# lmdu/pyfastx

Measured on NVIDIA B200. Metric: index_build_GBps, higher is better.
Workload: dtype u8

## Files before the change

pyfastx_b200/csrc/fxg_api.cu:

```cuda
#include "fxg_common.cuh"
#include <stdarg.h>
#include <stdlib.h>
#include <string.h>
#include <fcntl.h>
#include <unistd.h>
#include <sys/stat.h>
#include <sched.h>
#include <sys/mman.h>
#include <sys/syscall.h>
#include <thread>
#include <vector>
#include <atomic>
#include <mutex>

static thread_local char g_err[512] = "";

void fxg_set_error(const char *fmt, ...) {
    va_list ap;
    va_start(ap, fmt);
    vsnprintf(g_err, sizeof(g_err), fmt, ap);
    va_end(ap);
}

void fxg_pool_drain(int device);

int FxgScratch::reserve(size_t bytes) {
    if (bytes <= cap) return FXG_OK;
    if (ptr) cudaFree(ptr);
    ptr = nullptr; cap = 0;
    size_t want = bytes + bytes / 8 + 4096;
    cudaError_t e = cudaMalloc(&ptr, want);
    if (e != cudaSuccess) {
        cudaGetLastError();
        int dev = 0;
        cudaGetDevice(&dev);
        fxg_pool_drain(dev);
        want = bytes;
        e = cudaMalloc(&ptr, want);
    }
    if (e != cudaSuccess) {
        cudaGetLastError();
        ptr = nullptr;
        fxg_set_error("cudaMalloc(%zu) failed: %s", bytes, cudaGetErrorString(e));
        return FXG_ENOMEM;
    }
    cap = want;
    return FXG_OK;
}
void FxgScratch::release() {
    if (ptr) cudaFree(ptr);
    ptr = nullptr; cap = 0;
}

extern "C" int fxg_abi_version(void) { return FXG_ABI_VERSION; }
extern "C" const char *fxg_last_error(void) { return g_err; }

extern "C" int fxg_device_count(void) {
    int n = 0;
    if (cudaGetDeviceCount(&n) != cudaSuccess) { cudaGetLastError(); return 0; }
    return n;
}

static const size_t PINNED_CHUNK = (size_t)256 << 20;

extern "C" int fxg_ctx_create(int device, fxg_ctx **out) {
    FXG_CHECK_ARG(out, "out == NULL");
    *out = nullptr;
    int n = 0;
    cudaError_t e = cudaGetDeviceCount(&n);
    if (e != cudaSuccess || n == 0) {
        cudaGetLastError();
        fxg_set_error("no CUDA device available (%s); libfxg has no CPU fallback",
                      e != cudaSuccess ? cudaGetErrorString(e) : "device count 0");
        return FXG_ENODEV;
    }
    FXG_CHECK_ARG(device >= 0 && device < n, "device index out of range");
    FXG_CUDA(cudaSetDevice(device));
    cudaDeviceProp prop;
    FXG_CUDA(cudaGetDeviceProperties(&prop, device));
    if (prop.major < 10) {
        fxg_set_error("device %d is sm_%d%d; libfxg is built for sm_100a only", device, prop.major, prop.minor);
        return FXG_ENODEV;
    }
    if (const char *g = getenv("FXG_L2_FETCH")) {
        const int v = atoi(g);
        if (v == 32 || v == 64 || v == 128) cudaDeviceSetLimit(cudaLimitMaxL2FetchGranularity, (size_t)v);
    }
    fxg_ctx *c = new fxg_ctx();
    c->device = device;
    c->sm_count = prop.multiProcessorCount;
    FXG_CUDA(cudaStreamCreateWithFlags(&c->stream, cudaStreamNonBlocking));
    c->own_stream = true;
    *out = c;
    return FXG_OK;
}

void fxg_svc_stop(fxg_ctx *ctx);

extern "C" void fxg_ctx_destroy(fxg_ctx *c) {
    if (!c) return;
    cudaSetDevice(c->device);
    fxg_svc_stop(c);
    if (c->svc_stream) cudaStreamDestroy(c->svc_stream);
    if (c->svc_req) cudaFreeHost(c->svc_req);
    cudaStreamSynchronize(c->stream);
    if (c->h_counters) cudaFreeHost(c->h_counters);
    if (c->h_one) cudaFreeHost(c->h_one);
    if (c->ring) { cudaFreeHost(c->ring); for (int i = 0; i < 32; ++i) if (c->ring_ev[i]) cudaEventDestroy(c->ring_ev[i]); }
    for (int i = 0; i < 2; ++i) {
        if (c->pinned[i]) cudaFreeHost(c->pinned[i]);
        if (c->pinned_ev[i]) cudaEventDestroy(c->pinned_ev[i]);
    }
    for (int i = 0; i < FXG_PROF_SLOTS; ++i)
        for (int j = 0; j < 2; ++j) if (c->prof_ev[i][j]) cudaEventDestroy(c->prof_ev[i][j]);
    c->tile_desc.release(); c->seg.release(); c->cut.release(); c->row_tmp.release(); c->rows.release();
    c->counters.release(); c->params.release(); c->plan.release(); c->misc.release(); c->stage_file.release();
    if (c->own_stream && c->stream) cudaStreamDestroy(c->stream);
    delete c;
}

extern "C" int fxg_ctx_set_stream(fxg_ctx *c, void *cuda_stream) {
    FXG_CHECK_ARG(c, "ctx == NULL");
    FXG_LOCK(c);
    FXG_CUDA(cudaSetDevice(c->device));
    FXG_CUDA(cudaStreamSynchronize(c->stream));
    if (c->own_stream && c->stream) cudaStreamDestroy(c->stream);
    c->stream = (cudaStream_t)cuda_stream;
    c->own_stream = false;
    return FXG_OK;
}

extern "C" int fxg_ctx_sync(fxg_ctx *c) {
    FXG_CHECK_ARG(c, "ctx == NULL");
    FXG_LOCK(c);
    FXG_CUDA(cudaSetDevice(c->device));
    FXG_CUDA(cudaStreamSynchronize(c->stream));
    return FXG_OK;
}

extern "C" int fxg_ctx_sm_count(fxg_ctx *c) { return c ? c->sm_count : 0; }

extern "C" int fxg_profile_enable(fxg_ctx *c, int on) {
    FXG_CHECK_ARG(c, "ctx == NULL");
    FXG_LOCK(c);
    FXG_CUDA(cudaSetDevice(c->device));
    if (on && !c->prof_ev[0][0])
        for (int i = 0; i < FXG_PROF_SLOTS; ++i)
            for (int j = 0; j < 2; ++j) FXG_CUDA(cudaEventCreate(&c->prof_ev[i][j]));
    c->profiling = on != 0;
    for (int i = 0; i < FXG_PROF_SLOTS; ++i) c->prof_valid[i] = false;
    return FXG_OK;
}
extern "C" int fxg_profile_last_ms(fxg_ctx *c, int slot, float *ms) {
    FXG_CHECK_ARG(c && ms && slot >= 0 && slot < FXG_PROF_SLOTS, "bad arguments");
    FXG_LOCK(c);
    FXG_CHECK_ARG(c->prof_valid[slot], "no measurement recorded for this slot");
    FXG_CUDA(cudaEventSynchronize(c->prof_ev[slot][1]));
    FXG_CUDA(cudaEventElapsedTime(ms, c->prof_ev[slot][0], c->prof_ev[slot][1]));
    return FXG_OK;
}
extern "C" int64_t fxg_ctx_launch_count(fxg_ctx *c) { return c ? c->launches : 0; }

extern "C" int fxg_host_alloc(int64_t nbytes, void **out) {
    FXG_CHECK_ARG(out && nbytes >= 0, "bad arguments");
    *out = nullptr;
    FXG_CUDA(cudaHostAlloc(out, (size_t)(nbytes > 0 ? nbytes : 1), cudaHostAllocPortable));
    return FXG_OK;
}
extern "C" void fxg_host_free(void *p) {
    if (p) cudaFreeHost(p);
}

struct FxgFilePool {
    std::mutex mu;
    uint8_t *d[16] = {};
    int64_t cap[16] = {};
};
static FxgFilePool g_pool;
static bool pool_enabled() {
    static int on = -1;
    if (on < 0) { const char *e = getenv("FXG_FILE_POOL"); on = (e && e[0] == '0') ? 0 : 1; }
    return on != 0;
}
void fxg_pool_drain(int device) {
    std::lock_guard<std::mutex> g(g_pool.mu);
    for (int i = 0; i < 16; ++i)
        if ((device < 0 || device == i) && g_pool.d[i]) { cudaSetDevice(i); cudaFree(g_pool.d[i]); g_pool.d[i] = nullptr; g_pool.cap[i] = 0; }
}
extern "C" void fxg_pool_trim(void) { fxg_pool_drain(-1); }

extern "C" int fxg_file_alloc(fxg_ctx *c, int64_t nbytes, fxg_file **out) {
    FXG_CHECK_ARG(c && out && nbytes >= 0, "bad arguments");
    FXG_LOCK(c);
    *out = nullptr;
    FXG_CUDA(cudaSetDevice(c->device));
    fxg_file *f = new fxg_file();
    f->size = nbytes;
    f->capacity = fxg_round_up(nbytes + 1, FXG_FILE_PAD) + FXG_FILE_PAD;
    f->alloc_cap = f->capacity;
    f->owned = true;
    f->device = c->device;
    if (pool_enabled() && c->device < 16) {
        std::lock_guard<std::mutex> g(g_pool.mu);
        const int64_t have = g_pool.cap[c->device];
        if (g_pool.d[c->device] && have >= f->capacity && have <= 2 * f->capacity + ((int64_t)256 << 20)) {
            f->d = g_pool.d[c->device];
            f->alloc_cap = have;
            g_pool.d[c->device] = nullptr; g_pool.cap[c->device] = 0;
        }
    }
    if (f->d) {
        cudaDeviceSynchronize();
    } else {
        cudaError_t e = cudaMalloc((void **)&f->d, (size_t)f->capacity);
        if (e != cudaSuccess) {
            cudaGetLastError();
            fxg_pool_drain(c->device);
            e = cudaMalloc((void **)&f->d, (size_t)f->capacity);
        }
        if (e != cudaSuccess) {
            cudaGetLastError();
            delete f;
            fxg_set_error("cudaMalloc(%lld) for file buffer failed: %s", (long long)nbytes, cudaGetErrorString(e));
            return FXG_ENOMEM;
        }
    }
    const int64_t pad_from = nbytes & ~(int64_t)15;
    FXG_CUDA(cudaMemsetAsync(f->d + pad_from, 0, (size_t)(f->capacity - pad_from), c->stream));
    *out = f;
    return FXG_OK;
}

static bool host_ptr_is_pinned(const void *p) {
    cudaPointerAttributes a;
    if (cudaPointerGetAttributes(&a, p) != cudaSuccess) { cudaGetLastError(); return false; }
    return a.type == cudaMemoryTypeHost;
}

static int ensure_pinned(fxg_ctx *c) {
    if (c->pinned[0]) return FXG_OK;
    for (int i = 0; i < 2; ++i) {
        FXG_CUDA(cudaHostAlloc(&c->pinned[i], PINNED_CHUNK, cudaHostAllocDefault));
        FXG_CUDA(cudaEventCreateWithFlags(&c->pinned_ev[i], cudaEventDisableTiming));
    }
    c->pinned_bytes = PINNED_CHUNK;
    return FXG_OK;
}

static void parallel_memcpy(void *dst, const void *src, size_t n) {
    const size_t kMin = (size_t)4 << 20;
    unsigned nt = std::thread::hardware_concurrency();
    if (nt > 16) nt = 16;
    if (nt < 1) nt = 1;
    if (n < 2 * kMin || nt == 1) { memcpy(dst, src, n); return; }
    std::vector<std::thread> th;
    const size_t per = (n + nt - 1) / nt;
    for (unsigned i = 0; i < nt; ++i) {
        const size_t o = (size_t)i * per;
        if (o >= n) break;
        const size_t len = (o + per <= n) ? per : n - o;
        th.emplace_back([=] { memcpy((char *)dst + o, (const char *)src + o, len); });
    }
    for (auto &t : th) t.join();
}

extern "C" int fxg_file_upload(fxg_ctx *c, fxg_file *f, int64_t dst_off, const void *host, int64_t nbytes) {
    FXG_CHECK_ARG(c && f && (host || nbytes == 0), "bad arguments");
    FXG_LOCK(c);
    FXG_CHECK_ARG(dst_off >= 0 && nbytes >= 0 && dst_off + nbytes <= f->size, "upload range outside file");
    FXG_CUDA(cudaSetDevice(c->device));
    if (nbytes == 0) return FXG_OK;
    if (host_ptr_is_pinned(host)) {
        const int64_t chunk = (int64_t)256 << 20;
        for (int64_t o = 0; o < nbytes; o += chunk) {
            const int64_t len = (nbytes - o < chunk) ? nbytes - o : chunk;
            FXG_CUDA(cudaMemcpyAsync(f->d + dst_off + o, (const char *)host + o, (size_t)len,
                                     cudaMemcpyHostToDevice, c->stream));
        }
        return FXG_OK;
    }
    int rc = ensure_pinned(c);
    if (rc) return rc;
    int which = 0;
    for (int64_t o = 0; o < nbytes; o += (int64_t)c->pinned_bytes, which ^= 1) {
        const int64_t len = (nbytes - o < (int64_t)c->pinned_bytes) ? nbytes - o : (int64_t)c->pinned_bytes;
        FXG_CUDA(cudaEventSynchronize(c->pinned_ev[which]));
        parallel_memcpy(c->pinned[which], (const char *)host + o, (size_t)len);
        FXG_CUDA(cudaMemcpyAsync(f->d + dst_off + o, c->pinned[which], (size_t)len, cudaMemcpyHostToDevice, c->stream));
        FXG_CUDA(cudaEventRecord(c->pinned_ev[which], c->stream));
    }
    return FXG_OK;
}

extern "C" int fxg_file_from_host(fxg_ctx *c, const void *host, int64_t nbytes, fxg_file **out) {
    if (!c) { fxg_set_error("invalid argument: ctx == NULL"); return FXG_EINVAL; }
    FXG_LOCK(c);
    int rc = fxg_file_alloc(c, nbytes, out);
    if (rc) return rc;
    rc = fxg_file_upload(c, *out, 0, host, nbytes);
    if (rc) { fxg_file_free(*out); *out = nullptr; }
    return rc;
}

static int file_numa_node(int fd, int64_t begin, int64_t end) {
    if (end <= begin) return -1;
    const long pg = sysconf(_SC_PAGESIZE);
    int votes[64] = {0};
    int best = -1;
    const int64_t offs[3] = {begin / pg * pg, ((begin + end) / 2) / pg * pg, (end - 1) / pg * pg};
    for (int i = 0; i < 3; ++i) {
        void *m = mmap(nullptr, (size_t)pg, PROT_READ, MAP_SHARED, fd, (off_t)offs[i]);
        if (m == MAP_FAILED) continue;
        volatile char sink = *(volatile char *)m;
        (void)sink;
        int node = -1;
        if (syscall(SYS_get_mempolicy, &node, nullptr, 0ul, m, 3ul ) == 0 && node >= 0 && node < 64) {
            ++votes[node];
            if (best < 0 || votes[node] > votes[best]) best = node;
        }
        munmap(m, (size_t)pg);
    }
    return best;
}
static bool node_cpuset(int node, cpu_set_t *cs) {
    char pth[128], buf[4096];
    snprintf(pth, sizeof pth, "/sys/devices/system/node/node%d/cpulist", node);
    FILE *f = fopen(pth, "r");
    if (!f) return false;
    const bool got = fgets(buf, sizeof buf, f) != nullptr;
    fclose(f);
    if (!got) return false;
    CPU_ZERO(cs);
    int n = 0;
    for (char *p = buf; *p;) {
        char *e;
        long a = strtol(p, &e, 10);
        if (e == p) break;
        long b = a;
        if (*e == '-') { p = e + 1; b = strtol(p, &e, 10); }
        for (long c = a; c <= b && c < CPU_SETSIZE; ++c) { CPU_SET((int)c, cs); ++n; }
        p = (*e == ',') ? e + 1 : e;
        if (*e != ',' && *e != '-') break;
    }
    return n > 0;
}

static const int64_t RING_PIECE = (int64_t)16 << 20;
static const int RING_SLOTS = 32;
static int stage_path_range(fxg_ctx *c, const char *path, int64_t begin, int64_t end, fxg_file **out) {
    FXG_CHECK_ARG(c && path && out && begin >= 0, "bad arguments");
    *out = nullptr;
    int fd = open(path, O_RDONLY);
    if (fd < 0) { fxg_set_error("cannot open %s", path); return FXG_EIO; }
    struct stat st;
    if (fstat(fd, &st) != 0) { close(fd); fxg_set_error("cannot stat %s", path); return FXG_EIO; }
    if (end < 0 || end > (int64_t)st.st_size) end = (int64_t)st.st_size;
    if (begin > end) begin = end;
    const int64_t n = end - begin;
    int rc = fxg_file_alloc(c, n, out);
    if (rc) { close(fd); return rc; }
    if (!c->ring) {
        cudaError_t e = cudaHostAlloc(&c->ring, (size_t)(RING_PIECE * RING_SLOTS), cudaHostAllocDefault);
        if (e != cudaSuccess) { cudaGetLastError(); c->ring = nullptr; close(fd); fxg_file_free(*out); *out = nullptr; fxg_set_error("cudaHostAlloc of the staging ring failed: %s", cudaGetErrorString(e)); return FXG_ENOMEM; }
        for (int i = 0; i < RING_SLOTS; ++i) cudaEventCreateWithFlags(&c->ring_ev[i], cudaEventDisableTiming);
    }
    const int64_t np = (n + RING_PIECE - 1) / RING_PIECE;
    int nt = 20;
    if (const char *e = getenv("FXG_STAGE_THREADS")) { const int v = atoi(e); if (v >= 1 && v <= 256) nt = v; }
    const unsigned hw = std::thread::hardware_concurrency();
    if (hw && (unsigned)nt > hw) nt = (int)hw;
    if ((int64_t)nt > np) nt = (int)(np > 0 ? np : 1);
    cpu_set_t cs;
    bool pin = false;
    const char *pe = getenv("FXG_STAGE_PIN");
    if (!(pe && pe[0] == '0') && n >= ((int64_t)256 << 20)) {
        const int node = file_numa_node(fd, begin, end);
        pin = node >= 0 && node_cpuset(node, &cs);
        if (getenv("FXG_TIMING")) fprintf(stderr, "[fxg timing] staging: file pages on NUMA node %d, %d readers%s\n", node, nt, pin ? " pinned there" : "");
    }
    std::vector<std::atomic<int>> ready((size_t)(np > 0 ? np : 1));
    for (auto &r : ready) r.store(0, std::memory_order_relaxed);
    std::atomic<int64_t> next(0), retired_a(0);
    std::atomic<int> bad(0);
    char *ring = (char *)c->ring;
    std::vector<std::thread> th;
    for (int i = 0; i < nt && np > 0; ++i) th.emplace_back([&, pin] {
        if (pin) sched_setaffinity(0, sizeof(cs), &cs);
        for (;;) {
            const int64_t p = next.fetch_add(1);
            if (p >= np || bad.load(std::memory_order_relaxed)) return;
            while (p - retired_a.load(std::memory_order_acquire) >= RING_SLOTS) {
                if (bad.load(std::memory_order_relaxed)) return;
                std::this_thread::yield();
            }
            const int64_t o = p * RING_PIECE, len = n - o < RING_PIECE ? n - o : RING_PIECE;
            char *dst = ring + (p % RING_SLOTS) * RING_PIECE;
            int64_t done = 0;
            while (done < len) {
                const ssize_t r = pread(fd, dst + done, (size_t)(len - done), (off_t)(begin + o + done));
                if (r <= 0) { bad.store(1); return; }
                done += r;
            }
            ready[(size_t)p].store(1, std::memory_order_release);
        }
    });
    int64_t issued = 0, retired = 0;
    cudaError_t cerr = cudaSuccess;
    while (retired < np && !bad.load(std::memory_order_relaxed) && cerr == cudaSuccess) {
        bool progress = false;
        while (issued < np && ready[(size_t)issued].load(std::memory_order_acquire)) {
            const int64_t o = issued * RING_PIECE, len = n - o < RING_PIECE ? n - o : RING_PIECE;
            cerr = cudaMemcpyAsync((*out)->d + o, ring + (issued % RING_SLOTS) * RING_PIECE, (size_t)len, cudaMemcpyHostToDevice, c->stream);
            if (cerr != cudaSuccess) break;
            cudaEventRecord(c->ring_ev[issued % RING_SLOTS], c->stream);
            ++issued;
            progress = true;
        }
        while (retired < issued && cudaEventQuery(c->ring_ev[retired % RING_SLOTS]) == cudaSuccess) {
            ++retired;
            retired_a.store(retired, std::memory_order_release);
            progress = true;
        }
        if (!progress) std::this_thread::yield();
    }
    if (cerr != cudaSuccess) bad.store(1);
    for (auto &t : th) t.join();
    close(fd);
    cudaStreamSynchronize(c->stream);
    if (bad.load()) {
        cudaGetLastError();
        fxg_file_free(*out); *out = nullptr;
        if (cerr != cudaSuccess) { fxg_set_error("H2D failed: %s", cudaGetErrorString(cerr)); return FXG_ECUDA; }
        fxg_set_error("read error on %s", path);
        return FXG_EIO;
    }
    return FXG_OK;
}

extern "C" int fxg_file_from_path(fxg_ctx *c, const char *path, fxg_file **out) {
    FXG_CHECK_ARG(c, "ctx == NULL");
    FXG_LOCK(c);
    return stage_path_range(c, path, 0, -1, out);
}

extern "C" int fxg_file_from_path_range(fxg_ctx *c, const char *path, int64_t begin, int64_t end, fxg_file **out) {
    FXG_CHECK_ARG(c, "ctx == NULL");
    FXG_LOCK(c);
    return stage_path_range(c, path, begin, end, out);
}

extern "C" int fxg_file_slice(fxg_ctx *c, const fxg_file *src, int64_t begin, int64_t end, fxg_file **out) {
    FXG_CHECK_ARG(c && src && out && begin >= 0 && end >= begin && end <= src->size, "bad arguments");
    FXG_LOCK(c);
    int rc = fxg_file_alloc(c, end - begin, out);
    if (rc) return rc;
    if (end > begin)
        FXG_CUDA(cudaMemcpyAsync((*out)->d, src->d + begin, (size_t)(end - begin), cudaMemcpyDeviceToDevice, c->stream));
    return FXG_OK;
}

extern "C" int fxg_split_point_path(const char *path, int64_t from, int want_header, int64_t *pos, int64_t *file_size) {
    FXG_CHECK_ARG(path && pos && from >= 0, "bad arguments");
    int fd = open(path, O_RDONLY);
    if (fd < 0) { fxg_set_error("cannot open %s", path); return FXG_EIO; }
    struct stat st;
    if (fstat(fd, &st) != 0) { close(fd); fxg_set_error("cannot stat %s", path); return FXG_EIO; }
    const int64_t n = (int64_t)st.st_size;
    if (file_size) *file_size = n;
    *pos = n;
    if (from >= n) { close(fd); return FXG_OK; }
    std::vector<char> buf((size_t)1 << 20);
    if (from == 0) {
        char c0 = 0;
        if (!want_header || (pread(fd, &c0, 1, 0) == 1 && c0 == '>')) { *pos = 0; close(fd); return FXG_OK; }
        from = 1;
    }
    for (int64_t o = from - 1; o < n;) {
        const ssize_t got = pread(fd, buf.data(), buf.size(), (off_t)o);
        if (got <= 0) { close(fd); fxg_set_error("read error on %s", path); return FXG_EIO; }
        const char *b = buf.data();
        const char *p = b;
        const char *e = b + got;
        while ((p = (const char *)memchr(p, '\n', (size_t)(e - p))) != nullptr) {
            const int64_t x = o + (p - b);
            if (!want_header) { *pos = x + 1; close(fd); return FXG_OK; }
            if (p + 1 < e) {
                if (p[1] == '>') { *pos = x + 1; close(fd); return FXG_OK; }
            } else if (x + 1 < n) {
                char c1 = 0;
                if (pread(fd, &c1, 1, (off_t)(x + 1)) == 1 && c1 == '>') { *pos = x + 1; close(fd); return FXG_OK; }
            }
            ++p;
        }
        o += got;
    }
    close(fd);
    return FXG_OK;
}

extern "C" int fxg_file_wrap(fxg_ctx *c, void *dev_ptr, int64_t nbytes, int64_t capacity, fxg_file **out) {
    FXG_CHECK_ARG(c && out && dev_ptr && nbytes >= 0 && capacity >= nbytes, "bad arguments");
    FXG_LOCK(c);
    FXG_CHECK_ARG(((uintptr_t)dev_ptr & 15) == 0, "device pointer must be 16-byte aligned");
    FXG_CHECK_ARG(capacity >= fxg_round_up(nbytes, 16), "capacity must cover nbytes rounded up to 16");
    fxg_file *f = new fxg_file();
    f->d = (uint8_t *)dev_ptr; f->size = nbytes; f->capacity = capacity; f->owned = false; f->device = c->device;
    *out = f;
    return FXG_OK;
}

extern "C" int fxg_file_download(fxg_ctx *c, const fxg_file *f, int64_t src_off, void *host, int64_t nbytes) {
    FXG_CHECK_ARG(c && f && host && src_off >= 0 && nbytes >= 0 && src_off + nbytes <= f->size, "bad arguments");
    FXG_LOCK(c);
    FXG_CUDA(cudaSetDevice(c->device));
    FXG_CUDA(cudaMemcpyAsync(host, f->d + src_off, (size_t)nbytes, cudaMemcpyDeviceToHost, c->stream));
    FXG_CUDA(cudaStreamSynchronize(c->stream));
    return FXG_OK;
}

extern "C" void *fxg_file_devptr(const fxg_file *f) { return f ? f->d : nullptr; }
extern "C" int64_t fxg_file_size(const fxg_file *f) { return f ? f->size : 0; }
extern "C" void fxg_file_free(fxg_file *f) {
    if (!f) return;
    if (f->owned && f->d) {
        uint8_t *spare = f->d;
        int64_t cap = f->alloc_cap;
        if (pool_enabled() && f->device < 16 && cap >= ((int64_t)64 << 20)) {
            std::lock_guard<std::mutex> g(g_pool.mu);
            if (cap > g_pool.cap[f->device]) {
                std::swap(spare, g_pool.d[f->device]);
                std::swap(cap, g_pool.cap[f->device]);
            }
        }
        if (spare) { cudaSetDevice(f->device); cudaFree(spare); }
    }
    delete f;
}

extern "C" int fxg_rows_download(fxg_ctx *c, const void *d_rows, int64_t n_rows, int row_bytes, void *host_rows) {
    FXG_CHECK_ARG(c && (n_rows == 0 || (d_rows && host_rows)) && n_rows >= 0 && row_bytes > 0, "bad arguments");
    FXG_LOCK(c);
    FXG_CUDA(cudaSetDevice(c->device));
    if (n_rows) {
        FXG_CUDA(cudaMemcpyAsync(host_rows, d_rows, (size_t)n_rows * row_bytes, cudaMemcpyDeviceToHost, c->stream));
        FXG_CUDA(cudaStreamSynchronize(c->stream));
    }
    return FXG_OK;
}

extern "C" int fxg_rows_upload(fxg_ctx *c, const void *host_rows, int64_t n_rows, int row_bytes, void **d_rows_out) {
    FXG_CHECK_ARG(c && d_rows_out && n_rows >= 0 && row_bytes > 0 && (n_rows == 0 || host_rows), "bad arguments");
    FXG_LOCK(c);
    FXG_CUDA(cudaSetDevice(c->device));
    *d_rows_out = nullptr;
    void *d = nullptr;
    FXG_CUDA(cudaMalloc(&d, (size_t)(n_rows > 0 ? n_rows : 1) * row_bytes));
    if (n_rows) {
        cudaError_t e = cudaMemcpyAsync(d, host_rows, (size_t)n_rows * row_bytes, cudaMemcpyHostToDevice, c->stream);
        if (e == cudaSuccess) e = cudaStreamSynchronize(c->stream);
        if (e != cudaSuccess) { cudaFree(d); fxg_set_error("rows upload failed: %s", cudaGetErrorString(e)); return FXG_ECUDA; }
    }
    *d_rows_out = d;
    return FXG_OK;
}

extern "C" void fxg_dev_free(void *d) {
    if (d) cudaFree(d);
}

static int stage_into_ctx(fxg_ctx *c, const void *host_buf, int64_t nbytes, fxg_file *view) {
    FXG_CUDA(cudaSetDevice(c->device));
    const int64_t cap = fxg_round_up(nbytes + 1, FXG_FILE_PAD) + FXG_FILE_PAD;
    int rc = c->stage_file.reserve((size_t)cap);
    if (rc) return rc;
    view->d = (uint8_t *)c->stage_file.ptr;
    view->size = nbytes; view->capacity = cap; view->owned = false; view->device = c->device;
    const int64_t pad_from = nbytes & ~(int64_t)15;
    FXG_CUDA(cudaMemsetAsync(view->d + pad_from, 0, (size_t)(cap - pad_from), c->stream));
    return fxg_file_upload(c, view, 0, host_buf, nbytes);
}

extern "C" int fxg_fasta_build_index_host(fxg_ctx *c, const void *host_buf, int64_t nbytes, int flags,
                                          fxg_fasta_row *rows, int64_t rows_cap, fxg_scan_stats *stats) {
    FXG_CHECK_ARG(c && stats && (host_buf || nbytes == 0), "bad arguments");
    FXG_LOCK(c);
    fxg_file f;
    int rc = stage_into_ctx(c, host_buf, nbytes, &f);
    if (rc) return rc;
    fxg_fasta_row *d_rows = nullptr;
    rc = fxg_fasta_scan(c, &f, 0, flags, &d_rows, stats);
    if (rc == FXG_OK) {
        if (stats->n_rows > rows_cap) { fxg_set_error("rows_cap %lld < n_rows %lld", (long long)rows_cap, (long long)stats->n_rows); rc = FXG_ECAP; }
        else rc = fxg_rows_download(c, d_rows, stats->n_rows, (int)sizeof(fxg_fasta_row), rows);
    }
    return rc;
}

extern "C" int fxg_fastq_build_index_host(fxg_ctx *c, const void *host_buf, int64_t nbytes,
                                          fxg_fastq_row *rows, int64_t rows_cap, fxg_scan_stats *stats) {
    FXG_CHECK_ARG(c && stats && (host_buf || nbytes == 0), "bad arguments");
    FXG_LOCK(c);
    fxg_file f;
    int rc = stage_into_ctx(c, host_buf, nbytes, &f);
    if (rc) return rc;
    fxg_fastq_row *d_rows = nullptr;
    rc = fxg_fastq_scan(c, &f, 0, &d_rows, stats);
    if (rc == FXG_OK) {
        if (stats->n_rows > rows_cap) { fxg_set_error("rows_cap %lld < n_rows %lld", (long long)rows_cap, (long long)stats->n_rows); rc = FXG_ECAP; }
        else rc = fxg_rows_download(c, d_rows, stats->n_rows, (int)sizeof(fxg_fastq_row), rows);
    }
    return rc;
}
```

pyfastx_b200/csrc/fxg_common.cuh:

```cuda
#pragma once
#include <cuda_runtime.h>
#include <stdint.h>
#include <stdio.h>
#include <string>
#include <mutex>
#include "../../include/fxg.h"

void fxg_set_error(const char *fmt, ...);

#define FXG_CUDA(call)                                                                    \
    do {                                                                                  \
        cudaError_t e__ = (call);                                                         \
        if (e__ != cudaSuccess) {                                                         \
            fxg_set_error("%s failed: %s (%s:%d)", #call, cudaGetErrorString(e__),        \
                          __FILE__, __LINE__);                                            \
            return (e__ == cudaErrorNoDevice || e__ == cudaErrorInsufficientDriver)       \
                       ? FXG_ENODEV : (e__ == cudaErrorMemoryAllocation ? FXG_ENOMEM : FXG_ECUDA); \
        }                                                                                 \
    } while (0)

#define FXG_CHECK_ARG(cond, msg)                                                          \
    do {                                                                                  \
        if (!(cond)) { fxg_set_error("invalid argument: %s", msg); return FXG_EINVAL; }   \
    } while (0)

struct FxgScratch {
    void  *ptr = nullptr;
    size_t cap = 0;
    int reserve(size_t bytes);
    void release();
};

struct fxg_file {
    uint8_t *d = nullptr;
    int64_t  size = 0;
    int64_t  capacity = 0;
    int64_t  alloc_cap = 0;
    bool     owned = false;
    int      device = 0;
};

struct FxgScanRun {
    bool     active = false;
    int      mode = 0, flags = 0;
    const fxg_file *file = nullptr;
    int64_t  base_offset = 0;
};

struct fxg_ctx {
    std::recursive_mutex mu;
    FxgScanRun   run;
    int          device = 0;
    int          sm_count = 0;
    cudaStream_t stream = nullptr;
    bool         own_stream = false;
    void        *pinned[2] = {nullptr, nullptr};
    size_t       pinned_bytes = 0;
    cudaEvent_t  pinned_ev[2] = {nullptr, nullptr};
    void        *ring = nullptr;
    cudaEvent_t  ring_ev[32] = {};
    FxgScratch   tile_desc, seg, cut, row_tmp, rows, counters, params, plan, misc, stage_file;
    void        *h_counters = nullptr;
    void        *h_one = nullptr;
    void        *svc_req = nullptr, *svc_resp = nullptr;
    cudaStream_t svc_stream = nullptr;
    unsigned long long svc_next = 1;
    bool         svc_running = false;
    bool         profiling = false;
    cudaEvent_t  prof_ev[FXG_PROF_SLOTS][2] = {};
    bool         prof_valid[FXG_PROF_SLOTS] = {};
    int64_t      launches = 0;
    int64_t      collectives = 0;
};

#define FXG_LOCK(ctx) std::lock_guard<std::recursive_mutex> fxg_lock__((ctx)->mu)

struct FxgProfScope {
    fxg_ctx *c; int slot;
    FxgProfScope(fxg_ctx *ctx, int s, int nlaunch = 1) : c(ctx), slot(s) {
        c->launches += nlaunch;
        if (c->profiling) cudaEventRecord(c->prof_ev[slot][0], c->stream);
    }
    ~FxgProfScope() {
        if (c->profiling) { cudaEventRecord(c->prof_ev[slot][1], c->stream); c->prof_valid[slot] = true; }
    }
};

static const int64_t FXG_FILE_PAD = 65536;

inline int64_t fxg_round_up(int64_t v, int64_t m) { return (v + m - 1) / m * m; }

#ifdef __CUDACC__
namespace fxg {

__device__ __forceinline__ uint32_t smem_u32(const void *p) {
    return static_cast<uint32_t>(__cvta_generic_to_shared(p));
}
__device__ __forceinline__ void mbar_init(uint64_t *bar, uint32_t count) {
    asm volatile("mbarrier.init.shared::cta.b64 [%0], %1;" ::"r"(smem_u32(bar)), "r"(count));
}
__device__ __forceinline__ void mbar_fence_init() {
    asm volatile("fence.mbarrier_init.release.cluster;" ::: "memory");
}
__device__ __forceinline__ void mbar_expect_tx(uint64_t *bar, uint32_t bytes) {
    asm volatile("mbarrier.arrive.expect_tx.shared::cta.b64 _, [%0], %1;" ::"r"(smem_u32(bar)), "r"(bytes)
                 : "memory");
}
__device__ __forceinline__ void mbar_wait(uint64_t *bar, uint32_t parity) {
    asm volatile(
        "{\n\t"
        ".reg .pred p;\n\t"
        "WAIT_%=:\n\t"
        "mbarrier.try_wait.parity.shared::cta.b64 p, [%0], %1;\n\t"
        "@p bra DONE_%=;\n\t"
        "bra WAIT_%=;\n\t"
        "DONE_%=:\n\t"
        "}" ::"r"(smem_u32(bar)),
        "r"(parity)
        : "memory");
}
__device__ __forceinline__ void tma_load_1d(void *smem_dst, const void *gsrc, uint32_t bytes, uint64_t *bar) {
    asm volatile("cp.async.bulk.shared::cluster.global.mbarrier::complete_tx::bytes [%0], [%1], %2, [%3];" ::"r"(
                     smem_u32(smem_dst)),
                 "l"(gsrc), "r"(bytes), "r"(smem_u32(bar))
                 : "memory");
}
__device__ __forceinline__ void fence_proxy_async() {
    asm volatile("fence.proxy.async.shared::cta;" ::: "memory");
}

__device__ __forceinline__ uint32_t byte_eq_mask_r(uint32_t w, uint32_t c4, uint32_t k7f, uint32_t k80) {
    uint32_t u, r;
    asm("lop3.b32 %0, %1, %2, %3, 0x28;" : "=r"(u) : "r"(w), "r"(c4), "r"(k7f));
    const uint32_t t = u + k7f;
    asm("lop3.b32 %0, %1, %2, %3, 0x02;" : "=r"(r) : "r"(t), "r"(w), "r"(k80));
    return r;
}
__device__ __forceinline__ uint32_t byte_eq_mask(uint32_t w, uint32_t c4) {
    uint32_t u = (w ^ c4) & 0x7f7f7f7fu;
    uint32_t t = u + 0x7f7f7f7fu;
    return ~(t | w) & 0x80808080u;
}
__device__ __forceinline__ uint32_t chunk_eq_mask(const uint4 &v, uint32_t c4) {
    return byte_eq_mask(v.x, c4) | (byte_eq_mask(v.y, c4) >> 1) | (byte_eq_mask(v.z, c4) >> 2) |
           (byte_eq_mask(v.w, c4) >> 3);
}
__device__ __forceinline__ uint32_t chunk_eq_mask_r(const uint4 &v, uint32_t c4, uint32_t k7f, uint32_t k80) {
    return byte_eq_mask_r(v.x, c4, k7f, k80) | (byte_eq_mask_r(v.y, c4, k7f, k80) >> 1) |
           (byte_eq_mask_r(v.z, c4, k7f, k80) >> 2) | (byte_eq_mask_r(v.w, c4, k7f, k80) >> 3);
}
__device__ __forceinline__ uint32_t reg_const(uint32_t v) {
    uint32_t r;
    asm volatile("mov.b32 %0, %1;" : "=r"(r) : "r"(v));
    return r;
}
__device__ __forceinline__ int chunk_bit_to_off(int beta) { return ((7 - (beta & 7)) << 2) + (beta >> 3); }

__device__ __forceinline__ uint32_t ld_volatile_u32(const uint32_t *p) {
    uint32_t v;
    asm volatile("ld.volatile.global.u32 %0, [%1];" : "=r"(v) : "l"(p) : "memory");
    return v;
}
__device__ __forceinline__ void st_volatile_u32(uint32_t *p, uint32_t v) {
    asm volatile("st.volatile.global.u32 [%0], %1;" ::"l"(p), "r"(v) : "memory");
}
__device__ __forceinline__ int64_t ld_cg_i64(const int64_t *p) { return __ldcg(reinterpret_cast<const long long *>(p)); }
__device__ __forceinline__ uint64_t ld_cg_u64(const uint64_t *p) {
    return __ldcg(reinterpret_cast<const unsigned long long *>(p));
}

__device__ __forceinline__ int64_t shfl_i64(int64_t v, int src) {
    int lo = __shfl_sync(0xffffffffu, (int)(uint32_t)(uint64_t)v, src);
    int hi = __shfl_sync(0xffffffffu, (int)(uint32_t)((uint64_t)v >> 32), src);
    return (int64_t)(((uint64_t)(uint32_t)hi << 32) | (uint32_t)lo);
}
__device__ __forceinline__ int64_t shfl_up_i64(int64_t v, int d) {
    int lo = __shfl_up_sync(0xffffffffu, (int)(uint32_t)(uint64_t)v, d);
    int hi = __shfl_up_sync(0xffffffffu, (int)(uint32_t)((uint64_t)v >> 32), d);
    return (int64_t)(((uint64_t)(uint32_t)hi << 32) | (uint32_t)lo);
}
__device__ __forceinline__ int64_t shfl_down_i64(int64_t v, int d) {
    int lo = __shfl_down_sync(0xffffffffu, (int)(uint32_t)(uint64_t)v, d);
    int hi = __shfl_down_sync(0xffffffffu, (int)(uint32_t)((uint64_t)v >> 32), d);
    return (int64_t)(((uint64_t)(uint32_t)hi << 32) | (uint32_t)lo);
}

}
#endif
```

pyfastx_b200/csrc/fxg_scan.cu:

```cuda
#include "fxg_common.cuh"
#include <stdlib.h>
#include <string.h>
#include <limits.h>

namespace fxg {

#ifndef FXG_MARK_MINB
#define FXG_MARK_MINB 6
#endif
constexpr int REGION   = 2048;
constexpr int SEGCAP   = 128;
constexpr int MARK_WARPS = 8;
constexpr int PS_THREADS = 256, PS_PER_THREAD = 16, PS_BLOCK = PS_THREADS * PS_PER_THREAD;
constexpr int64_t NOPOS = INT64_MIN / 4;
constexpr uint32_t E_POS = 0x07ffu, E_CR = 1u << 14, E_HDR = 1u << 15;

struct __align__(16) FastaTmp {
    int64_t  boff;
    int64_t  lineidx;
    int64_t  llen;
    uint64_t S;
    uint64_t evmax;
    uint64_t evminc;
    uint32_t D;
    int32_t  dlen;
    int32_t  nlen;
    uint32_t elen;
};
static_assert(sizeof(FastaTmp) == 64, "FastaTmp layout");

struct ScanTotals {
    uint64_t nl;
    uint64_t hdr;
    int64_t  n_eff;
    uint64_t sum_len;
    int64_t  lead_lines, lead_bytes, lead_llen;
    int64_t  first_line;
    int64_t  nrows;
    int64_t  row0;
    int64_t  n_owned;
    int64_t  total_lines;
    int64_t  pad[4];
};
static_assert(sizeof(ScanTotals) == 128, "ScanTotals layout");
static_assert(sizeof(fxg_shard_info) == 128, "fxg_shard_info layout");

struct ScanParams;
struct ScanParams {
    const uint8_t *file;
    int64_t   n;
    int64_t   capacity;
    int64_t   nreg;
    int64_t   base_offset;
    int64_t   first_line;
    int       flags;
    uint2    *rc;
    uint4    *rec2;
    uint16_t *seg;
    uint8_t  *cut;
    ulonglong2 *ex;
    ulonglong2 *bs;
    ScanTotals *totals;
    FastaTmp *tmp;
    int64_t   tmp_cap;
    fxg_fastq_row *qrows;
    int64_t   qrows_cap;
    const ScanParams *self;
};

__device__ __forceinline__ uint4 ld_stream16(const uint8_t *p) {
    uint4 v;
    asm volatile("ld.global.nc.L1::no_allocate.v4.u32 {%0, %1, %2, %3}, [%4];"
                 : "=r"(v.x), "=r"(v.y), "=r"(v.z), "=r"(v.w) : "l"(p));
    return v;
}

#ifndef FXG_MARK_CUT
#define FXG_MARK_CUT 0
#endif
#ifndef FXG_CUT_WORDS
#define FXG_CUT_WORDS 6
#endif
__device__ __forceinline__ uint32_t swz_unit(uint32_t u);
template <int V> __device__ __forceinline__ uint32_t region_byte(const uint8_t *sb, uint32_t p);
template <int V>
__device__ __forceinline__ uint32_t name_cut_smem(const uint8_t *sb, uint32_t a) {
    uint32_t M = 0;
#pragma unroll
    for (int k = 0; k < FXG_CUT_WORDS; ++k) {
        const uint32_t wq = min((a >> 2) + (uint32_t)k, (uint32_t)(REGION / 4 - 1));
        const uint32_t w = reinterpret_cast<const uint32_t *>(sb)[V == 2 ? ((swz_unit(wq >> 2) << 2) | (wq & 3u)) : wq];
        const uint32_t lt = ~((((w & 0x7f7f7f7fu) + 0x5f5f5f5fu) | w)) & 0x80808080u;
        M |= ((lt * 0x00204081u) >> 28) << (4 * k);
    }
    M &= 0xffffffffu << (a & 3u);
    if (!M) return 255u;
    const uint32_t p = (a & ~3u) + (uint32_t)(__ffs(M) - 1);
    if (p >= (uint32_t)REGION) return 255u;
    if (p >= ((a >> 2) + (uint32_t)FXG_CUT_WORDS) * 4u) return 255u;
    const uint32_t b = region_byte<V>(sb, p);
    if (b == ' ') return p - a;
    if (b == '\n' || b == 0u) return 254u;
    if (b == '\r' && p + 1u < (uint32_t)REGION && region_byte<V>(sb, p + 1u) == '\n') return 254u;
    return 255u;
}

#ifndef FXG_MARK_V_FASTA
#define FXG_MARK_V_FASTA 1
#endif
#ifndef FXG_MARK_V_FASTQ
#define FXG_MARK_V_FASTQ 2
#endif
#ifndef FXG_MARK_RPW
#define FXG_MARK_RPW 1
#endif
__device__ __forceinline__ uint32_t swz_unit(uint32_t u) { return u ^ ((u >> 3) & 7u); }
template <int V>
__device__ __forceinline__ uint32_t region_byte(const uint8_t *sb, uint32_t p) {
    return V == 2 ? sb[(swz_unit(p >> 4) << 4) | (p & 15u)] : sb[p];
}

template <int MODE, int V>
__global__ void __launch_bounds__(MARK_WARPS * 32, FXG_MARK_MINB) mark_kernel(const ScanParams P) {
    __shared__ uint4    s_data[MARK_WARPS * (REGION / 16) + (FXG_MARK_CUT ? 2 : 0)];
    __shared__ uint16_t s_ent[MARK_WARPS][SEGCAP];
    const int lane = threadIdx.x & 31, warp = threadIdx.x >> 5;
    const int64_t r0 = ((int64_t)blockIdx.x * MARK_WARPS + warp) * FXG_MARK_RPW;
    if (r0 >= P.nreg) return;
    const uint32_t lt_mask = (1u << lane) - 1u;
    const int64_t n = P.n;
    const uint8_t *file = P.file;
    const uint32_t k0a = reg_const(0x0a0a0a0au), k7f = reg_const(0x7f7f7f7fu), k80 = reg_const(0x80808080u);

    auto load_region = [&](int64_t rr, uint4 (&vv)[4]) {
        const int64_t base = rr * REGION;
        if (base + REGION <= n) {
            const uint8_t *src = file + base + lane * 16;
#pragma unroll
            for (int j = 0; j < 4; ++j) vv[j] = ld_stream16(src + j * 512);
        } else {
#pragma unroll
            for (int j = 0; j < 4; ++j) {
                const int64_t o = base + j * 512 + lane * 16;
                if (o + 16 <= n) { vv[j] = ld_stream16(file + o); continue; }
                const bool virt = n > 0 && file[n - 1] != '\n';
                uint32_t w[4] = {0, 0, 0, 0};
                for (int i = 0; i < 16; ++i) {
                    const int64_t x = o + i;
                    const uint32_t b = x < n ? file[x] : ((virt && x == n) ? 0x0au : 0u);
                    w[i >> 2] |= b << ((i & 3) * 8);
                }
                vv[j] = make_uint4(w[0], w[1], w[2], w[3]);
            }
        }
    };
    uint4 vn[4];
    load_region(r0, vn);
#pragma unroll 1
    for (int it = 0; it < FXG_MARK_RPW; ++it) {
    const int64_t r = r0 + it;
    if (r >= P.nreg) break;
    const int64_t base = r * REGION;
    uint4 v[4] = {vn[0], vn[1], vn[2], vn[3]};
    if (it + 1 < FXG_MARK_RPW && r + 1 < P.nreg) load_region(r + 1, vn);
    uint32_t nlc = 0;
    uint16_t *ent = s_ent[warp];

    if constexpr (V == 2) {
    uint4 *sd = s_data + warp * (REGION / 16);
#pragma unroll
    for (int j = 0; j < 4; ++j) sd[swz_unit((uint32_t)(j * 32 + lane))] = v[j];
    __syncwarp();
    uint32_t lo = 0, hi = 0;
#pragma unroll
    for (int i = 0; i < 4; ++i) {
        const uint4 x = sd[swz_unit((uint32_t)(4 * lane + i))];
        const uint32_t w4[4] = {x.x, x.y, x.z, x.w};
#pragma unroll
        for (int c = 0; c < 4; ++c) {
            const uint32_t f = byte_eq_mask_r(w4[c], k0a, k7f, k80);
            const uint32_t nib = (f * 0x00204081u) >> 28;
            const int k = 4 * i + c;
            if (k < 8) lo = nib * (1u << (4 * k)) + lo;
            else hi = nib * (1u << (4 * (k - 8))) + hi;
        }
    }
    {
        const uint32_t c = (uint32_t)(__popc(lo) + __popc(hi));
        const uint32_t b1 = __ballot_sync(0xffffffffu, c >= 1u), b2 = __ballot_sync(0xffffffffu, c >= 2u);
        const uint32_t b3 = __ballot_sync(0xffffffffu, c >= 3u);
        const uint32_t pbase = (uint32_t)lane * 64u;
        if (!b3) {
            const uint32_t idx = (uint32_t)(__popc(b1 & lt_mask) + __popc(b2 & lt_mask));
            nlc = (uint32_t)(__popc(b1) + __popc(b2));
            if (c) {
                const uint32_t p1 = lo ? (uint32_t)(__ffs(lo) - 1) : 32u + (uint32_t)(__ffs(hi) - 1);
                if (idx < (uint32_t)SEGCAP) ent[idx] = (uint16_t)(pbase + p1);
                if (c >= 2u) {
                    if (lo) lo &= lo - 1u; else hi &= hi - 1u;
                    const uint32_t p2 = lo ? (uint32_t)(__ffs(lo) - 1) : 32u + (uint32_t)(__ffs(hi) - 1);
                    if (idx + 1u < (uint32_t)SEGCAP) ent[idx + 1u] = (uint16_t)(pbase + p2);
                }
            }
        } else {
            uint32_t incl = c;
#pragma unroll
            for (int d = 1; d < 32; d <<= 1) {
                const uint32_t o2 = __shfl_up_sync(0xffffffffu, incl, d);
                if (lane >= d) incl += o2;
            }
            nlc = __shfl_sync(0xffffffffu, incl, 31);
            uint32_t idx = incl - c;
            while (lo) { if (idx < (uint32_t)SEGCAP) ent[idx] = (uint16_t)(pbase + (uint32_t)(__ffs(lo) - 1)); lo &= lo - 1u; ++idx; }
            while (hi) { if (idx < (uint32_t)SEGCAP) ent[idx] = (uint16_t)(pbase + 32u + (uint32_t)(__ffs(hi) - 1)); hi &= hi - 1u; ++idx; }
        }
    }
    __syncwarp();
    } else {
    uint32_t m[4];
    int cmax = 0;
#pragma unroll
    for (int j = 0; j < 4; ++j) {
        s_data[warp * (REGION / 16) + j * 32 + lane] = v[j];
        m[j] = chunk_eq_mask_r(v[j], k0a, k7f, k80);
        cmax = max(cmax, __popc(m[j]));
    }
    const bool any2 = __any_sync(0xffffffffu, cmax >= 2);
    const bool multi = any2 && __any_sync(0xffffffffu, cmax >= 3);
    if (!any2) {
#pragma unroll
        for (int j = 0; j < 4; ++j) {
            const uint32_t bn = __ballot_sync(0xffffffffu, m[j] != 0);
            if (m[j]) {
                const uint32_t idx = nlc + __popc(bn & lt_mask);
                if (idx < (uint32_t)SEGCAP) ent[idx] = (uint16_t)(j * 512 + lane * 16 + chunk_bit_to_off(__ffs(m[j]) - 1));
            }
            nlc += __popc(bn);
        }
    } else if (!multi) {
#pragma unroll
        for (int j = 0; j < 4; ++j) {
            const int c = __popc(m[j]);
            const uint32_t bn1 = __ballot_sync(0xffffffffu, c >= 1);
            const uint32_t bn2 = __ballot_sync(0xffffffffu, c >= 2);
            if (c) {
                const uint32_t idx = nlc + __popc(bn1 & lt_mask) + __popc(bn2 & lt_mask);
                const int xo = j * 512 + lane * 16;
                int oa = chunk_bit_to_off(__ffs(m[j]) - 1);
                if (c == 2) {
                    const uint32_t m2 = m[j] & (m[j] - 1);
                    const int ob = chunk_bit_to_off(__ffs(m2) - 1);
                    const int hi = max(oa, ob);
                    oa = min(oa, ob);
                    if (idx + 1 < (uint32_t)SEGCAP) ent[idx + 1] = (uint16_t)(xo + hi);
                }
                if (idx < (uint32_t)SEGCAP) ent[idx] = (uint16_t)(xo + oa);
            }
            nlc += __popc(bn1) + __popc(bn2);
        }
    }
    if (multi) {
        nlc = 0;
#pragma unroll 1
        for (int j = 0; j < 4; ++j) {
            uint32_t mj = 0;
#pragma unroll
            for (int jj = 0; jj < 4; ++jj) if (jj == j) mj = m[jj];
            const uint32_t c = (uint32_t)__popc(mj);
            uint32_t incl = c;
#pragma unroll
            for (int d = 1; d < 32; d <<= 1) {
                const uint32_t o2 = __shfl_up_sync(0xffffffffu, incl, d);
                if (lane >= d) incl += o2;
            }
            uint32_t idx = nlc + incl - c;
#pragma unroll 1
            for (int w = 0; w < 4; ++w) {
                uint32_t mw = mj & (0x80808080u >> w);
                while (mw) {
                    if (idx < (uint32_t)SEGCAP) ent[idx] = (uint16_t)(j * 512 + lane * 16 + chunk_bit_to_off(__ffs(mw) - 1));
                    mw &= mw - 1;
                    ++idx;
                }
            }
            nlc += __shfl_sync(0xffffffffu, incl, 31);
        }
    }
    __syncwarp();
    }

    const uint8_t *sb = reinterpret_cast<const uint8_t *>(s_data + warp * (REGION / 16));
    uint32_t hc = 0;
    if (nlc <= (uint32_t)SEGCAP) {
        uint16_t *dst = P.seg + r * SEGCAP;
        const uint32_t nround = (nlc + 15u) & ~15u;
        uint32_t imask = 0, hmask = 0;
        for (uint32_t k0 = 0; k0 < nround; k0 += 32) {
            const uint32_t k = k0 + lane;
            uint32_t e = 0, cutv = 255u;
            if (k < nlc) {
                const uint32_t pos = ent[k];
                e = pos;
                if (FXG_MARK_CUT && MODE == 1 && pos + 2u < (uint32_t)REGION && region_byte<V>(sb, pos + 1u) == '@') cutv = name_cut_smem<V>(sb, pos + 2u);
                if (MODE == 0) {
                    const uint32_t next = pos < (uint32_t)(REGION - 1) ? region_byte<V>(sb, pos + 1u)
                                                                      : (base + REGION < n ? (uint32_t)file[base + REGION] : 0u);
                    if (next == '>') e |= E_HDR;
                } else {
                    const uint32_t prev = pos > 0 ? region_byte<V>(sb, pos - 1u) : (base > 0 ? (uint32_t)file[base - 1] : 0u);
                    if (prev == '\r') e |= E_CR;
                }
            }
            if (MODE == 0) {
                const uint32_t hb = __ballot_sync(0xffffffffu, (e & E_HDR) != 0);
                hc += __popc(hb);
                if (k0 == 0) {
                    const uint32_t e1 = __shfl_up_sync(0xffffffffu, e, 1), e2 = __shfl_up_sync(0xffffffffu, e, 2);
                    const bool it = lane >= 2 && k < nlc &&
                                    (((e1 | e2) & E_HDR) != 0 || (e & E_POS) - (e1 & E_POS) != (e1 & E_POS) - (e2 & E_POS));
                    imask = __ballot_sync(0xffffffffu, it);
                    hmask = hb;
                }
            }
            if (k < nround) dst[k] = (uint16_t)e;
            if (FXG_MARK_CUT && MODE == 1) P.cut[r * SEGCAP + k] = (uint8_t)cutv;
            if (k < nlc) ent[k] = (uint16_t)e;
        }
        __syncwarp();
        if (lane == 0) {
            const uint32_t last = nlc >= 1 ? ent[nlc - 1] : 0u, prev = nlc >= 2 ? ent[nlc - 2] : 0u;
            P.rc[r] = make_uint2(nlc | (hc << 16), last | (prev << 16));
            if (MODE == 0) {
                const uint32_t f0 = nlc >= 1 ? ent[0] : 0u, f1 = nlc >= 2 ? ent[1] : 0u;
                P.rec2[r] = make_uint4(f0 | (f1 << 16), nlc > 32u ? 0xffffffffu : imask, hmask, 0u);
            }
        }
    } else {
        if (MODE == 0) {
            uint32_t myh = 0;
            for (int x = lane; x < REGION; x += 32)
                if (region_byte<V>(sb, (uint32_t)x) == '\n') {
                    const uint32_t next = x < REGION - 1 ? region_byte<V>(sb, (uint32_t)x + 1u) : (base + REGION < n ? (uint32_t)file[base + REGION] : 0u);
                    myh += next == '>';
                }
            hc = __reduce_add_sync(0xffffffffu, myh);
        }
        if (lane == 0) {
            P.rc[r] = make_uint2(nlc | (hc << 16), 0u);
            if (MODE == 0) P.rec2[r] = make_uint4(0u, 0xffffffffu, 0u, 0u);
        }
    }
    __syncwarp();
    }
}

__global__ void __launch_bounds__(PS_THREADS) prefix_reduce_kernel(const uint2 *rc, ulonglong2 *bs) {
    __shared__ uint32_t sm[16];
    const uint4 *p = reinterpret_cast<const uint4 *>(rc + (size_t)blockIdx.x * PS_BLOCK + (size_t)threadIdx.x * PS_PER_THREAD);
    uint32_t a = 0, b = 0;
#pragma unroll
    for (int i = 0; i < PS_PER_THREAD / 2; ++i) {
        const uint4 q = p[i];
        a += (q.x & 0xffffu) + (q.z & 0xffffu);
        b += (q.x >> 16) + (q.z >> 16);
    }
    a = __reduce_add_sync(0xffffffffu, a);
    b = __reduce_add_sync(0xffffffffu, b);
    const int lane = threadIdx.x & 31, warp = threadIdx.x >> 5;
    if (lane == 0) { sm[warp] = a; sm[8 + warp] = b; }
    __syncthreads();
    if (threadIdx.x == 0) {
        uint64_t ta = 0, tb = 0;
        for (int w = 0; w < PS_THREADS / 32; ++w) { ta += sm[w]; tb += sm[8 + w]; }
        bs[blockIdx.x] = make_ulonglong2(ta, tb);
    }
}

__global__ void __launch_bounds__(1024) prefix_blocks_kernel(ulonglong2 *bs, int64_t nb, const uint8_t *file, int64_t n,
                                                             int mode, ScanTotals *tot) {
    __shared__ uint64_t s_a[32], s_b[32];
    __shared__ uint64_t s_ca, s_cb;
    const int lane = threadIdx.x & 31, warp = threadIdx.x >> 5;
    if (threadIdx.x == 0) { s_ca = 0; s_cb = (mode == 0 && n > 0 && file[0] == '>') ? 1u : 0u; }
    __syncthreads();
    for (int64_t b0 = 0; b0 < nb; b0 += 1024) {
        const int64_t i = b0 + threadIdx.x;
        const ulonglong2 v = i < nb ? bs[i] : make_ulonglong2(0, 0);
        uint64_t a = v.x, b = v.y;
#pragma unroll
        for (int d = 1; d < 32; d <<= 1) {
            const uint64_t oa = (uint64_t)shfl_up_i64((int64_t)a, d), ob = (uint64_t)shfl_up_i64((int64_t)b, d);
            if (lane >= d) { a += oa; b += ob; }
        }
        if (lane == 31) { s_a[warp] = a; s_b[warp] = b; }
        __syncthreads();
        uint64_t wa = 0, wb = 0;
        for (int w = 0; w < warp; ++w) { wa += s_a[w]; wb += s_b[w]; }
        const uint64_t ca = s_ca, cb = s_cb;
        if (i < nb) bs[i] = make_ulonglong2(ca + wa + a - v.x, cb + wb + b - v.y);
        __syncthreads();
        if (threadIdx.x == 1023) { s_ca = ca + wa + a; s_cb = cb + wb + b; }
        __syncthreads();
    }
    if (threadIdx.x == 0) {
        const bool virt = n > 0 && file[n - 1] != '\n';
        tot->nl = s_ca; tot->hdr = s_cb; tot->n_eff = n + (virt ? 1 : 0);
    }
}

__global__ void __launch_bounds__(PS_THREADS) prefix_expand_kernel(const uint2 *rc, const ulonglong2 *bs, ulonglong2 *ex,
                                                                 int64_t nreg) {
    __shared__ uint32_t s_a[PS_THREADS / 32], s_b[PS_THREADS / 32];
    const int lane = threadIdx.x & 31, warp = threadIdx.x >> 5;
    const size_t r0 = (size_t)blockIdx.x * PS_BLOCK + (size_t)threadIdx.x * PS_PER_THREAD;
    const uint4 *p = reinterpret_cast<const uint4 *>(rc + r0);
    uint32_t c[PS_PER_THREAD];
    uint32_t a = 0, b = 0;
#pragma unroll
    for (int i = 0; i < PS_PER_THREAD / 2; ++i) {
        const uint4 q = p[i];
        c[2 * i] = q.x; c[2 * i + 1] = q.z;
        a += (q.x & 0xffffu) + (q.z & 0xffffu);
        b += (q.x >> 16) + (q.z >> 16);
    }
    uint32_t ia = a, ib = b;
#pragma unroll
    for (int d = 1; d < 32; d <<= 1) {
        const uint32_t oa = __shfl_up_sync(0xffffffffu, ia, d), ob = __shfl_up_sync(0xffffffffu, ib, d);
        if (lane >= d) { ia += oa; ib += ob; }
    }
    if (lane == 31) { s_a[warp] = ia; s_b[warp] = ib; }
    __syncthreads();
    uint32_t wa = 0, wb = 0;
    for (int w = 0; w < warp; ++w) { wa += s_a[w]; wb += s_b[w]; }
    const ulonglong2 bb = bs[blockIdx.x];
    uint64_t ea = bb.x + wa + ia - a, eb = bb.y + wb + ib - b;
#pragma unroll
    for (int i = 0; i < PS_PER_THREAD; ++i) {
        if ((int64_t)(r0 + i) < nreg) ex[r0 + i] = make_ulonglong2(ea, eb);
        ea += c[i] & 0xffffu; eb += c[i] >> 16;
    }
}

__device__ __forceinline__ int64_t find_first_of2(const uint8_t *h, int64_t limit, uint32_t a4, uint32_t b4, int *which) {
    const int mis = (int)((uintptr_t)h & 3);
    const uint32_t *wp = reinterpret_cast<const uint32_t *>(h - mis);
    *which = 0;
    for (int64_t k = -mis; k < limit; k += 16, wp += 4) {
        const uint32_t w0 = wp[0], w1 = wp[1], w2 = wp[2], w3 = wp[3];
        uint32_t ma[4] = {byte_eq_mask(w0, a4), byte_eq_mask(w1, a4), byte_eq_mask(w2, a4), byte_eq_mask(w3, a4)};
        uint32_t mb[4] = {byte_eq_mask(w0, b4), byte_eq_mask(w1, b4), byte_eq_mask(w2, b4), byte_eq_mask(w3, b4)};
#pragma unroll
        for (int i = 0; i < 4; ++i) {
            uint32_t m = ma[i] | mb[i];
            const int64_t kk = k + 4 * i;
            if (kk < 0) m &= 0xffffffffu << (8 * (int)(-kk));
            if (m) {
                const int byte = (__ffs(m) - 1) >> 3;
                const int64_t pos = kk + byte;
                if (pos >= limit) return limit;
                *which = ((mb[i] >> (8 * byte)) & 0x80u) ? 2 : 1;
                return pos;
            }
        }
    }
    return limit;
}

struct Prev2 {
    int64_t  pos1, pos0;
    uint32_t h1, h0;
};

template <int MODE>
__device__ __forceinline__ uint32_t is_hdr_at(const ScanParams &P, int64_t x) {
    return (MODE == 0 && x < P.n && P.file[x] == '>') ? 1u : 0u;
}
__device__ __forceinline__ bool nl_at(const ScanParams &P, int64_t x) {
    return x < P.n ? P.file[x] == '\n' : (x == P.n && P.n > 0 && P.file[P.n - 1] != '\n');
}

template <int MODE>
__device__ __forceinline__ void do_line(const ScanParams &P, int64_t first_line, int64_t p, int64_t pm1, int64_t pm2, bool h1, bool h2,
                                        int64_t hcount, int64_t lineidx, bool cr, unsigned long long &my_size) {
    const uint8_t *file = P.file;
    const int64_t s = pm1 + 1;
    const int64_t L = p - pm1;
    if (MODE == 0) {
        const int64_t slot = hcount;
        if (h1) {
            const int elen = (p >= 1 && (p - 1 < P.n ? file[p - 1] : 0) == '\r') ? 2 : 1;
            const int64_t dlen = L - 1 - elen;
            int64_t nlen = dlen;
            if (!(P.flags & FXG_SCAN_FULL_NAME)) {
                nlen = 0;
                if (s + 1 + dlen + 20 <= P.capacity) {
                    int which;
                    nlen = find_first_of2(file + s + 1, dlen, 0x20202020u, 0x09090909u, &which);
                } else {
                    while (nlen < dlen) {
                        const uint8_t ch = file[s + 1 + nlen];
                        if (ch == ' ' || ch == '\t') break;
                        ++nlen;
                    }
                }
            }
            if (slot < P.tmp_cap) {
                FastaTmp *t = &P.tmp[slot];
                t->boff = P.base_offset + p + 1;
                t->lineidx = lineidx;
                t->dlen = (int32_t)dlen;
                t->nlen = (int32_t)nlen;
                t->elen = (uint32_t)elen;
            }
        } else if (slot < P.tmp_cap) {
            const bool prev_exists = pm1 >= 0;
            if (!prev_exists || h2) {
                P.tmp[slot].llen = L;
            } else {
                const int64_t prevL = pm1 - pm2;
                if (L != prevL) {
                    FastaTmp *t = &P.tmp[slot];
                    atomicAdd(&t->D, 1u);
                    atomicMax((unsigned long long *)&t->evmax, (unsigned long long)lineidx);
                    atomicMax((unsigned long long *)&t->evminc, ~(unsigned long long)lineidx);
                    atomicAdd((unsigned long long *)&t->S, (unsigned long long)(L - prevL));
                }
            }
        }
    } else {
        const int64_t gline = first_line + lineidx;
        const int ph = (int)(gline & 3);
        const int64_t row = (gline >> 2) - (first_line >> 2);
        const int64_t len = L - 1;
        if (ph == 1) {
            const int64_t rlen = (len > 0 && cr) ? len - 1 : len;
            my_size += (unsigned long long)rlen;
            if (row < P.qrows_cap) { P.qrows[row].soff = P.base_offset + s; P.qrows[row].rlen = rlen; }
        } else if (row < P.qrows_cap) {
            if (ph == 0) {
                int64_t l = len - 1;
                if (l > 0 && cr) --l;
                if (l < 0) l = 0;
                int64_t k = 0;
                if (s + 1 + l + 20 <= P.capacity) {
                    int which;
                    k = find_first_of2(file + s + 1, l, 0x20202020u, 0x00000000u, &which);
                    if (which == 2) k = l;
                } else {
                    for (; k < l; ++k) {
                        const uint8_t ch = file[s + 1 + k];
                        if (ch == 0) { k = l; break; }
                        if (ch == ' ') break;
                    }
                }
                *reinterpret_cast<int2 *>(&P.qrows[row].dlen) = make_int2((int)len, (int)k);
            } else if (ph == 3) {
                P.qrows[row].qoff = P.base_offset + s;
            }
        }
    }
}

template <int MODE>
__device__ __noinline__ Prev2 carry_walk(const ScanParams *Pg, int64_t r) {
    const ScanParams &P = *Pg;
    Prev2 cy;
    const int lane = threadIdx.x & 31;
    cy.pos1 = cy.pos0 = NOPOS; cy.h1 = cy.h0 = 0;
    int need = 2;
    auto push = [&](int64_t pos, uint32_t h) {
        if (need == 2) { cy.pos1 = pos; cy.h1 = h; } else { cy.pos0 = pos; cy.h0 = h; }
        --need;
    };
    int64_t q = r - 1;
    while (need > 0 && q >= 0) {
        const int64_t qq = q - lane;
        const uint32_t c = qq >= 0 ? (P.rc[qq].x & 0xffffu) : 0u;
        const uint32_t nz = __ballot_sync(0xffffffffu, c != 0);
        if (!nz) { q -= 32; continue; }
        const int f = __ffs(nz) - 1;
        q -= f;
        const int cq = (int)__shfl_sync(0xffffffffu, c, f);
        if (cq <= SEGCAP) {
            const uint16_t *sg = P.seg + q * SEGCAP;
            for (int i = cq - 1; i >= 0 && need > 0; --i) {
                const uint32_t e = sg[i];
                push(q * REGION + (int64_t)(e & E_POS), MODE == 0 ? (e >> 15) : 0u);
            }
        } else {
            for (int64_t x = q * REGION + REGION - 1; x >= q * REGION && need > 0; --x)
                if (nl_at(P, x)) push(x, is_hdr_at<MODE>(P, x + 1));
        }
        q -= 1;
    }
    if (need > 0) push(-1, is_hdr_at<MODE>(P, 0));
    return cy;
}

template <int MODE>
__device__ __noinline__ unsigned long long dense_region(const ScanParams *Pg, int64_t first_line, int64_t r, Prev2 cy,
                                                        ulonglong2 exv) {
    const ScanParams &P = *Pg;
    unsigned long long my_size = 0;
    const int lane = threadIdx.x & 31;
    const uint8_t *file = P.file;
    const int64_t b0 = r * REGION + lane * 64;
    uint32_t c = 0, h = 0;
    Prev2 inc; inc.pos1 = inc.pos0 = NOPOS; inc.h1 = inc.h0 = 0;
    for (int i = 0; i < 64; ++i) {
        const int64_t x = b0 + i;
        if (nl_at(P, x)) {
            const uint32_t hh = is_hdr_at<MODE>(P, x + 1);
            ++c; h += hh;
            inc.pos0 = inc.pos1; inc.h0 = inc.h1; inc.pos1 = x; inc.h1 = hh;
        }
    }
    uint32_t ic = c, ih = h;
    uint32_t icnt = c > 2 ? 2 : c;
#pragma unroll
    for (int d = 1; d < 32; d <<= 1) {
        const uint32_t oc = __shfl_up_sync(0xffffffffu, ic, d), oh = __shfl_up_sync(0xffffffffu, ih, d);
        const int64_t op1 = shfl_up_i64(inc.pos1, d), op0 = shfl_up_i64(inc.pos0, d);
        const uint32_t oh1 = __shfl_up_sync(0xffffffffu, inc.h1, d), oh0 = __shfl_up_sync(0xffffffffu, inc.h0, d);
        const uint32_t ocnt = __shfl_up_sync(0xffffffffu, icnt, d);
        if (lane >= d) {
            ic += oc; ih += oh;
            if (icnt == 0) { inc.pos1 = op1; inc.h1 = oh1; inc.pos0 = op0; inc.h0 = oh0; icnt = ocnt; }
            else if (icnt == 1 && ocnt >= 1) { inc.pos0 = op1; inc.h0 = oh1; icnt = 2; }
        }
    }
    Prev2 pv;
    pv.pos1 = shfl_up_i64(inc.pos1, 1); pv.pos0 = shfl_up_i64(inc.pos0, 1);
    pv.h1 = __shfl_up_sync(0xffffffffu, inc.h1, 1); pv.h0 = __shfl_up_sync(0xffffffffu, inc.h0, 1);
    uint32_t pcnt = __shfl_up_sync(0xffffffffu, icnt, 1);
    if (lane == 0) pcnt = 0;
    if (pcnt == 0) pv = cy;
    else if (pcnt == 1) { pv.pos0 = cy.pos1; pv.h0 = cy.h1; }
    int64_t idx = (int64_t)exv.x + (ic - c);
    int64_t hcount = (int64_t)exv.y + (ih - h);
    for (int i = 0; i < 64 && c; ++i) {
        const int64_t x = b0 + i;
        if (!nl_at(P, x)) continue;
        const bool cr = x > 0 && file[x - 1] == '\r';
        do_line<MODE>(P, first_line, x, pv.pos1, pv.pos0, pv.h1 != 0, pv.h0 != 0, hcount, idx, cr, my_size);
        const uint32_t hh = is_hdr_at<MODE>(P, x + 1);
        hcount += hh; ++idx;
        pv.pos0 = pv.pos1; pv.h0 = pv.h1; pv.pos1 = x; pv.h1 = hh;
    }
    return my_size;
}

template <int MODE>
__device__ __forceinline__ void region_batches(const ScanParams &P, int64_t first_line, int64_t r, int nl, Prev2 cy, ulonglong2 X,
                                               uint32_t E0, uint32_t E1, unsigned long long &my_size) {
    const int lane = threadIdx.x & 31;
    const uint32_t lt_mask = (1u << lane) - 1u;
    const int64_t base = r * REGION;
    const uint16_t *sg = P.seg + r * SEGCAP;
    int64_t hrun = (int64_t)X.y;
    for (int k0 = 0; k0 < nl; k0 += 32) {
        const int k = k0 + lane;
        const bool valid = k < nl;
        uint32_t e = k0 == 0 ? E0 : (k0 == 32 ? E1 : (valid ? (uint32_t)sg[k] : 0u));
        if (!valid) e = 0;
        const uint32_t hb = __ballot_sync(0xffffffffu, (e & E_HDR) != 0);
        const uint32_t e1 = __shfl_up_sync(0xffffffffu, e, 1), e2 = __shfl_up_sync(0xffffffffu, e, 2);
        if (valid) {
            int64_t pm1, pm2;
            bool h1, h2;
            if (lane >= 1) { pm1 = base + (e1 & E_POS); h1 = (e1 & E_HDR) != 0; } else { pm1 = cy.pos1; h1 = cy.h1 != 0; }
            if (lane >= 2) { pm2 = base + (e2 & E_POS); h2 = (e2 & E_HDR) != 0; }
            else if (lane == 1) { pm2 = cy.pos1; h2 = cy.h1 != 0; }
            else { pm2 = cy.pos0; h2 = cy.h0 != 0; }
            do_line<MODE>(P, first_line, base + (e & E_POS), pm1, pm2, h1, h2, hrun + __popc(hb & lt_mask), (int64_t)X.x + k,
                          (e & E_CR) != 0, my_size);
        }
        const uint32_t l31 = __shfl_sync(0xffffffffu, e, 31), l30 = __shfl_sync(0xffffffffu, e, 30);
        cy.pos1 = base + (l31 & E_POS); cy.h1 = (l31 >> 15) & 1u;
        cy.pos0 = base + (l30 & E_POS); cy.h0 = (l30 >> 15) & 1u;
        hrun += __popc(hb);
    }
}

template <int MODE>
__device__ __noinline__ unsigned long long full_region(const ScanParams *Pg, int64_t first_line, int64_t r) {
    const ScanParams &P = *Pg;
    unsigned long long my_size = 0;
    const int lane = threadIdx.x & 31;
    const int nl = (int)(P.rc[r].x & 0xffffu);
    if (nl == 0) return 0;
    const ulonglong2 X = P.ex[r];
    Prev2 cy = carry_walk<MODE>(Pg, r);
    if (MODE != 0) cy.h1 = cy.h0 = 0;
    if (nl <= SEGCAP) region_batches<MODE>(P, first_line, r, nl, cy, X, P.seg[r * SEGCAP + lane], P.seg[r * SEGCAP + 32 + lane], my_size);
    else my_size += dense_region<MODE>(Pg, first_line, r, cy, X);
    return my_size;
}

constexpr int LG = 4;

template <int MODE>
__global__ void __launch_bounds__(MARK_WARPS * 32) lines_kernel(const ScanParams P) {
    const int64_t first_line = MODE == 1 ? P.totals->first_line : 0;
    const int lane = threadIdx.x & 31;
    const int64_t r0 = ((int64_t)blockIdx.x * MARK_WARPS + (threadIdx.x >> 5)) * LG;
    if (r0 >= P.nreg) return;
    unsigned long long my_size = 0;

    const int64_t rq = r0 + (LG - 1) - lane;
    const uint2 A = rq >= 0 ? P.rc[rq] : make_uint2(0u, 0u);
    ulonglong2 X[LG];
    uint32_t E[LG][2];
#pragma unroll
    for (int i = 0; i < LG; ++i) {
        const int64_t r = r0 + i;
        X[i] = make_ulonglong2(0, 0); E[i][0] = E[i][1] = 0;
        if (r < P.nreg) {
            X[i] = P.ex[r];
            E[i][0] = P.seg[r * SEGCAP + lane];
            E[i][1] = P.seg[r * SEGCAP + 32 + lane];
        }
    }
    const uint32_t cntl = A.x & 0xffffu;
    const uint32_t nzall = __ballot_sync(0xffffffffu, cntl != 0);
    const bool window_hits_start = r0 + (LG - 1) - 31 <= 0;

#pragma unroll
    for (int i = 0; i < LG; ++i) {
        const int64_t r = r0 + i;
        const int me = LG - 1 - i;
        const int nl = (int)__shfl_sync(0xffffffffu, cntl, me);
        if (nl == 0) continue;

        Prev2 cy;
        cy.pos1 = cy.pos0 = NOPOS; cy.h1 = cy.h0 = 0;
        {
            bool slow = false;
            const uint32_t nz = nzall & ~((2u << me) - 1u);
            if (nz) {
                const int f1 = __ffs(nz) - 1;
                const uint32_t n1 = __shfl_sync(0xffffffffu, cntl, f1), y1 = __shfl_sync(0xffffffffu, A.y, f1);
                const int64_t b1 = (r0 + (LG - 1) - f1) * REGION;
                if (n1 > (uint32_t)SEGCAP) slow = true;
                else {
                    cy.pos1 = b1 + (y1 & E_POS); cy.h1 = (y1 >> 15) & 1u;
                    if (n1 >= 2) { cy.pos0 = b1 + ((y1 >> 16) & E_POS); cy.h0 = y1 >> 31; }
                    else {
                        const uint32_t nz2 = nz & ~(1u << f1);
                        if (nz2) {
                            const int f2 = __ffs(nz2) - 1;
                            const uint32_t n2 = __shfl_sync(0xffffffffu, cntl, f2), y2 = __shfl_sync(0xffffffffu, A.y, f2);
                            if (n2 > (uint32_t)SEGCAP) slow = true;
                            else { cy.pos0 = (r0 + (LG - 1) - f2) * REGION + (y2 & E_POS); cy.h0 = (y2 >> 15) & 1u; }
                        } else if (window_hits_start) { cy.pos0 = -1; cy.h0 = is_hdr_at<MODE>(P, 0); }
                        else slow = true;
                    }
                }
            } else if (window_hits_start) { cy.pos1 = -1; cy.h1 = is_hdr_at<MODE>(P, 0); }
            else slow = true;
            if (slow) cy = carry_walk<MODE>(P.self, r);
            if (MODE != 0) cy.h1 = cy.h0 = 0;
        }
        if (nl <= SEGCAP) region_batches<MODE>(P, first_line, r, nl, cy, X[i], E[i][0], E[i][1], my_size);
        else my_size += dense_region<MODE>(P.self, first_line, r, cy, X[i]);
    }

    if (MODE == 1) {
#pragma unroll
        for (int d = 16; d > 0; d >>= 1) my_size += (unsigned long long)shfl_down_i64((int64_t)my_size, d);
        if (lane == 0 && my_size) atomicAdd((unsigned long long *)&P.totals->sum_len, my_size);
    }
}

#ifndef FXG_FQ_PRELOAD
#define FXG_FQ_PRELOAD 0
#endif
#ifndef FXG_FQ_PAIRSTORE
#define FXG_FQ_PAIRSTORE 1
#endif
constexpr int RG = 8;
constexpr int RWIN = RG + 2;
static_assert(RWIN * REGION <= 32768, "window positions must fit 15 bits");

__global__ void __launch_bounds__(MARK_WARPS * 32) fastq_records_kernel(const ScanParams Pin) {
    __shared__ uint16_t s_flat[MARK_WARPS][RWIN * SEGCAP];
    __shared__ uint8_t  s_cut[MARK_WARPS][FXG_MARK_CUT ? RWIN * SEGCAP : 1];
    const ScanParams &P = Pin;
    const int64_t first_line = Pin.totals->first_line;
    const int lane = threadIdx.x & 31, warp = threadIdx.x >> 5;
    const int64_t r0 = ((int64_t)blockIdx.x * MARK_WARPS + warp) * RG;
    if (r0 >= P.nreg) return;
    unsigned long long my_size = 0;
    const uint8_t *file = P.file;

    const int64_t rl = r0 - 1 + lane;
    uint2 rec = make_uint2(0u, 0u);
    uint64_t exl = 0;
    if (lane <= RWIN && rl >= 0 && rl < P.nreg) { rec = P.rc[rl]; exl = P.ex[rl].x; }
    const uint32_t nll = rec.x & 0xffffu;
    const uint32_t densem = __ballot_sync(0xffffffffu, nll > (uint32_t)SEGCAP);
    if (densem & (((1u << RG) - 1u) << 1)) {
        for (int i = 0; i < RG; ++i)
            if (r0 + i < P.nreg) my_size += full_region<1>(P.self, first_line, r0 + i);
    } else {
        const uint64_t ex0 = (uint64_t)shfl_i64((int64_t)exl, 1);
        uint16_t *flat = s_flat[warp];
        uint8_t *cutf = s_cut[warp];
        uint32_t E2[RWIN];
#pragma unroll
        for (int i = 0; i < RWIN; ++i) {
            E2[i] = 0u;
            if (FXG_FQ_PRELOAD && r0 + i < P.nreg) E2[i] = reinterpret_cast<const uint32_t *>(P.seg + (r0 + i) * SEGCAP)[lane];
        }
        int W = 0, Ls = 0;
        bool closed = false;
#pragma unroll
        for (int i = 0; i < RWIN; ++i) {
            const int nl = (int)__shfl_sync(0xffffffffu, nll, i + 1);
            if (nl > SEGCAP) closed = true;
            if (!closed) {
                const int k = 2 * lane;
                if (!FXG_FQ_PRELOAD && k < nl) E2[i] = reinterpret_cast<const uint32_t *>(P.seg + (r0 + i) * SEGCAP)[lane];
                const uint32_t e0 = E2[i] & 0xffffu, e1 = E2[i] >> 16;
                if (k < nl) flat[W + k] = (uint16_t)((i * REGION + (int)(e0 & E_POS)) | ((e0 & E_CR) ? 0x8000u : 0u));
                if (k + 1 < nl) flat[W + k + 1] = (uint16_t)((i * REGION + (int)(e1 & E_POS)) | ((e1 & E_CR) ? 0x8000u : 0u));
                if (nl > 64) {
                    const uint16_t *sg = P.seg + (r0 + i) * SEGCAP;
                    for (int kk = 64 + lane; kk < nl; kk += 32) {
                        const uint32_t e = sg[kk];
                        flat[W + kk] = (uint16_t)((i * REGION + (int)(e & E_POS)) | ((e & E_CR) ? 0x8000u : 0u));
                    }
                }
                if (FXG_MARK_CUT) {
                    const uint8_t *cg = P.cut + (r0 + i) * SEGCAP;
                    for (int kk = lane; kk < nl; kk += 32) cutf[W + kk] = cg[kk];
                }
                W += nl;
            }
            if (i == RG - 1) Ls = W;
        }
        __syncwarp();
        int64_t carry;
        uint32_t carry_cut = 255u;
        {
            const uint32_t pn = __shfl_sync(0xffffffffu, nll, 0), py = __shfl_sync(0xffffffffu, rec.y, 0);
            if (r0 == 0) carry = -1;
            else if (pn >= 1 && pn <= (uint32_t)SEGCAP) {
                carry = (r0 - 1) * REGION + (int64_t)(py & E_POS);
                if (FXG_MARK_CUT) carry_cut = P.cut[(r0 - 1) * SEGCAP + (pn - 1)];
            } else carry = carry_walk<1>(P.self, r0).pos1;
        }
        const int64_t span_base = r0 * REGION;
        auto POS = [&](int f) -> int64_t { return f < 0 ? carry : span_base + (int64_t)(flat[f] & 0x7fffu); };
        auto CR = [&](int f) -> bool { return (flat[f] & 0x8000u) != 0; };
        const int64_t g0 = first_line + (int64_t)ex0;
        const int64_t row0 = first_line >> 2;
        int lead = (int)((4 - (g0 & 3)) & 3);
        if (lead > Ls) lead = Ls;
        if (lane < lead) {
            const int f = lane;
            const int64_t g = g0 + f;
            const int ph = (int)(g & 3);
            const int64_t row = (g >> 2) - row0;
            const int64_t pm1 = POS(f - 1), p = POS(f);
            if (ph == 1) {
                const int64_t len = p - pm1 - 1;
                const int64_t rlen = (len > 0 && CR(f)) ? len - 1 : len;
                my_size += (unsigned long long)rlen;
                if (row < P.qrows_cap) { P.qrows[row].soff = P.base_offset + pm1 + 1; P.qrows[row].rlen = rlen; }
            } else if (ph == 3) {
                if (row < P.qrows_cap) P.qrows[row].qoff = P.base_offset + pm1 + 1;
            }
        }
        for (int fb = lead; fb < Ls; fb += 128) {
            const int f = fb + 4 * lane;
            int64_t row = 0, soff = 0, rlen = 0, qoff = 0, len = 0, k = 0;
            bool have1 = false, have3 = false;
            const bool mine = f < Ls;
            if (mine) {
                row = ((g0 + f) >> 2) - row0;
                have1 = f + 1 < W; have3 = f + 3 < W;
                const int64_t pm1 = POS(f - 1), p0 = POS(f);
                len = p0 - pm1 - 1;
                int64_t l = len - 1;
                if (l > 0 && CR(f)) --l;
                if (l < 0) l = 0;
                const int64_t s = pm1 + 1;
                const uint32_t cv = !FXG_MARK_CUT ? 255u : (f >= 1 ? (uint32_t)cutf[f - 1] : carry_cut);
                if (cv < 254u) k = (int64_t)cv < l ? (int64_t)cv : l;
                else if (cv == 254u) k = l;
                else if (s + 1 + l + 20 <= P.capacity) {
                    int which;
                    k = find_first_of2(file + s + 1, l, 0x20202020u, 0x00000000u, &which);
                    if (which == 2) k = l;
                } else {
                    for (; k < l; ++k) {
                        const uint8_t ch = file[s + 1 + k];
                        if (ch == 0) { k = l; break; }
                        if (ch == ' ') break;
                    }
                }
                if (have1) {
                    const int64_t p1 = POS(f + 1);
                    const int64_t len1 = p1 - p0 - 1;
                    soff = P.base_offset + p0 + 1;
                    rlen = (len1 > 0 && CR(f + 1)) ? len1 - 1 : len1;
                    if (f + 1 < Ls) my_size += (unsigned long long)rlen;
                }
                if (have3) qoff = P.base_offset + POS(f + 2) + 1;
            }
            const bool full = mine && have3 && row < P.qrows_cap;
            const int other_full = __shfl_xor_sync(0xffffffffu, full ? 1 : 0, 1);
            const bool pair_full = FXG_FQ_PAIRSTORE && full && other_full != 0;
            longlong2 a, b;
            a.x = soff; a.y = qoff;
            b.x = rlen; b.y = (long long)(((unsigned long long)(uint32_t)(int)k << 32) | (uint32_t)(int)len);
            const bool odd = (lane & 1) != 0;
            const longlong2 send = odd ? a : b;
            longlong2 recv;
            recv.x = shfl_i64(send.x, lane ^ 1);
            recv.y = shfl_i64(send.y, lane ^ 1);
            if (pair_full) {
                fxg_fastq_row *q0 = &P.qrows[odd ? row - 1 : row];
                reinterpret_cast<longlong2 *>(q0)[odd ? 1 : 0] = odd ? recv : a;
                reinterpret_cast<longlong2 *>(q0 + 1)[odd ? 1 : 0] = odd ? b : recv;
            } else if (mine && row < P.qrows_cap) {
                fxg_fastq_row *q = &P.qrows[row];
                if (have3) {
                    reinterpret_cast<longlong2 *>(q)[0] = a;
                    reinterpret_cast<longlong2 *>(q)[1] = b;
                } else {
                    *reinterpret_cast<int2 *>(&q->dlen) = make_int2((int)len, (int)k);
                    if (have1) { q->soff = soff; q->rlen = rlen; }
                }
            }
        }
    }
#pragma unroll
    for (int d = 16; d > 0; d >>= 1) my_size += (unsigned long long)shfl_down_i64((int64_t)my_size, d);
    if (lane == 0 && my_size) atomicAdd((unsigned long long *)&P.totals->sum_len, my_size);
}

__global__ void __launch_bounds__(MARK_WARPS * 32) fasta_lines_kernel(const ScanParams P) {
    const int lane = threadIdx.x & 31;
    const int64_t R0 = ((int64_t)blockIdx.x * MARK_WARPS + (threadIdx.x >> 5)) * 32;
    if (R0 >= P.nreg) return;
    const int64_t r = R0 + lane;
    const bool inb = r < P.nreg;
    unsigned long long dummy = 0;
    uint2 me = make_uint2(0u, 0u), pv = make_uint2(0u, 0u);
    uint4 q = make_uint4(0u, 0u, 0u, 0u);
    ulonglong2 X = make_ulonglong2(0, 0);
    if (inb) {
        me = P.rc[r];
        if (r >= 1) pv = P.rc[r - 1];
        q = P.rec2[r];
        X = P.ex[r];
    }
    const uint32_t nl = me.x & 0xffffu, pnl = pv.x & 0xffffu;
    const bool full = nl != 0 && (nl > 32u || r == 0 || pnl < 2u || pnl > (uint32_t)SEGCAP || q.y == 0xffffffffu);
    uint32_t mask = 0;
    const uint32_t c1 = pv.y & 0xffffu, c0 = pv.y >> 16, f0 = q.x & 0xffffu, f1 = q.x >> 16;
    if (nl != 0 && !full) {
        const int p_c1 = (int)(c1 & E_POS) - REGION, p_c0 = (int)(c0 & E_POS) - REGION;
        const int p_f0 = (int)(f0 & E_POS), p_f1 = (int)(f1 & E_POS);
        const int L0 = p_f0 - p_c1;
        const bool i0 = ((c1 | c0) & E_HDR) != 0 || L0 != p_c1 - p_c0;
        const bool i1 = nl >= 2u && (((f0 | c1) & E_HDR) != 0 || p_f1 - p_f0 != L0);
        mask = (q.y & ~3u) | (i0 ? 1u : 0u) | (i1 ? 2u : 0u);
        if (nl < 32u) mask &= (1u << nl) - 1u;
    }
    const int64_t base = r * REGION;
    const uint16_t *sg = P.seg + r * SEGCAP;
    while (mask) {
        const int k = __ffs(mask) - 1;
        mask &= mask - 1;
        uint32_t e, m1, m2;
        int64_t b1 = base, b2 = base;
        if (k >= 2) { e = sg[k]; m1 = sg[k - 1]; m2 = sg[k - 2]; }
        else if (k == 1) { e = f1; m1 = f0; m2 = c1; b2 = base - REGION; }
        else { e = f0; m1 = c1; m2 = c0; b1 = b2 = base - REGION; }
        do_line<0>(P, 0, base + (e & E_POS), b1 + (m1 & E_POS), b2 + (m2 & E_POS), (m1 & E_HDR) != 0, (m2 & E_HDR) != 0,
                   (int64_t)X.y + __popc(q.z & ((1u << k) - 1u)), (int64_t)X.x + k, false, dummy);
    }
    uint32_t fm = __ballot_sync(0xffffffffu, full);
    while (fm) {
        const int f = __ffs(fm) - 1;
        fm &= fm - 1;
        full_region<0>(P.self, 0, R0 + f);
    }
}


__global__ void __launch_bounds__(256) fasta_finalize_kernel(const FastaTmp *tmp, int64_t tmp_cap, int64_t rows_cap,
                                                             int64_t base_offset, ScanTotals *tot, fxg_fasta_row *rows) {
    int64_t nrows = (int64_t)tot->hdr;
    if (nrows > rows_cap || nrows + 1 > tmp_cap) nrows = 0;
    unsigned long long slen_acc = 0;
    const int64_t stride = (int64_t)gridDim.x * blockDim.x;
    for (int64_t r = (int64_t)blockIdx.x * blockDim.x + threadIdx.x; r < nrows; r += stride) {
        const FastaTmp t = tmp[r + 1];
        int64_t next_h, next_line;
        if (r + 1 < nrows) {
            const FastaTmp nx = tmp[r + 2];
            next_h = nx.boff - (1 + nx.dlen + (int64_t)nx.elen);
            next_line = nx.lineidx;
        } else {
            next_h = base_offset + tot->n_eff;
            next_line = (int64_t)tot->nl;
        }
        const int64_t blen = next_h - t.boff;
        const int64_t nlines = next_line - t.lineidx - 1;
        const int64_t slen = blen - nlines * (int64_t)t.elen;
        int norm;
        if (t.D == 0) norm = 1;
        else if (t.D == 1) norm = ((int64_t)t.evmax == t.lineidx + nlines) ? 1 : 0;
        else if (t.D == 2) norm = ((t.evmax - (~t.evminc) == 1) && t.S == 0) ? 1 : 0;
        else norm = 0;
        fxg_fasta_row o;
        o.boff = t.boff; o.blen = blen; o.slen = slen; o.llen = t.llen;
        o.dlen = t.dlen; o.nlen = t.nlen; o.elen = (uint8_t)t.elen; o.norm = (uint8_t)norm;
        for (int i = 0; i < 6; ++i) o.pad[i] = 0;
        o.pad[0] = (t.D == 0 || (t.D == 1 && (int64_t)t.evmax == t.lineidx + nlines && (int64_t)t.S < 0)) ? 1 : 0;
        rows[r] = o;
        slen_acc += (unsigned long long)slen;
    }
#pragma unroll
    for (int d = 16; d > 0; d >>= 1) slen_acc += (unsigned long long)shfl_down_i64((int64_t)slen_acc, d);
    if ((threadIdx.x & 31) == 0 && slen_acc) atomicAdd((unsigned long long *)&tot->sum_len, slen_acc);
    if (blockIdx.x == 0 && threadIdx.x == 0) {
        const FastaTmp l = tmp[0];
        tot->lead_llen = l.llen;
        if (nrows > 0) {
            const FastaTmp f = tmp[1];
            tot->lead_lines = f.lineidx;
            tot->lead_bytes = f.boff - base_offset - (1 + f.dlen + (int64_t)f.elen);
        }
    }
}

__global__ void __launch_bounds__(32) edge_kernel(const ScanParams P, int mode, fxg_shard_info *info) {
    const int lane = threadIdx.x;
    int found = 0;
    int64_t pos[3] = {0, 0, 0};
    for (int64_t r0 = 0; r0 < P.nreg && found < 3; r0 += 32) {
        const int64_t r = r0 + lane;
        const uint32_t c = r < P.nreg ? (P.rc[r].x & 0xffffu) : 0u;
        uint32_t nz = __ballot_sync(0xffffffffu, c != 0);
        while (nz && found < 3) {
            const int fl = __ffs(nz) - 1;
            nz &= nz - 1;
            const int64_t q = r0 + fl;
            const int cq = (int)__shfl_sync(0xffffffffu, c, fl);
            if (cq <= SEGCAP) {
                for (int i = 0; i < cq && found < 3; ++i) pos[found++] = q * REGION + (int64_t)(P.seg[q * SEGCAP + i] & E_POS);
            } else {
                for (int64_t x = q * REGION; x < q * REGION + REGION && found < 3; ++x)
                    if (nl_at(P, x)) pos[found++] = x;
            }
        }
    }
    if (lane == 0) {
        const ScanTotals t = *P.totals;
        fxg_shard_info o;
        o.n_rows = mode == 0 ? (int64_t)t.hdr : 0;
        o.n_lines = (int64_t)t.nl;
        o.bytes = P.n;
        o.base_offset = P.base_offset;
        o.end_position = t.n_eff;
        o.edge_n = found;
        int64_t start = 0;
        for (int j = 0; j < 3; ++j) {
            o.edge_off[j] = 0; o.edge_len[j] = 0;
            if (j < found) {
                const int64_t p = pos[j];
                const bool cr = p > start && p - 1 < P.n && P.file[p - 1] == '\r';
                o.edge_off[j] = P.base_offset + start;
                o.edge_len[j] = p - start - (cr ? 1 : 0);
                start = p + 1;
            }
        }
        for (int j = 0; j < 4; ++j) o.reserved[j] = 0;
        *info = o;
    }
}

__global__ void shard_prefix_kernel(const fxg_shard_info *all, int nranks, int rank, int mode, ScanTotals *tot) {
    if (threadIdx.x != 0 || blockIdx.x != 0) return;
    int64_t F = 0, T = 0;
    for (int p = 0; p < nranks; ++p) {
        const int64_t nlp = all[p].n_lines;
        if (p < rank) F += nlp;
        T += nlp;
    }
    if (mode == 0) F = 0;
    tot->first_line = F;
    tot->total_lines = T;
    const int64_t nl = (int64_t)tot->nl;
    tot->nrows = mode == 0 ? (int64_t)tot->hdr : (F + nl + 3) / 4 - F / 4;
    tot->sum_len = 0;
}

__global__ void __launch_bounds__(256) clear_kernel(const ScanParams P, int mode, int64_t tmp_slots) {
    const int64_t nrows = P.totals->nrows;
    const int64_t stride = (int64_t)gridDim.x * blockDim.x;
    const int64_t t0 = (int64_t)blockIdx.x * blockDim.x + threadIdx.x;
    if (mode == 0) {
        int64_t slots = nrows + 2;
        if (slots > tmp_slots) slots = tmp_slots;
        uint4 *p = reinterpret_cast<uint4 *>(P.tmp);
        for (int64_t i = t0; i < slots * 4; i += stride) p[i] = make_uint4(0u, 0u, 0u, 0u);
    } else if (t0 < 4) {
        const int64_t row = t0 < 2 ? 0 : nrows - 1;
        if (row >= 0 && row < P.qrows_cap) reinterpret_cast<uint4 *>(P.qrows + row)[t0 & 1] = make_uint4(0u, 0u, 0u, 0u);
    }
}

__global__ void fastq_stitch_kernel(const ScanParams P, const fxg_shard_info *all, int nranks, int rank) {
    if (threadIdx.x != 0 || blockIdx.x != 0) return;
    ScanTotals *tot = P.totals;
    const int64_t F = tot->first_line, n = (int64_t)tot->nl, T = tot->total_lines;
    const int64_t first_read = (F + 3) / 4;
    int64_t last_read = n > 0 ? (F + n - 1) / 4 : first_read - 1;
    if (last_read > T / 4 - 1) last_read = T / 4 - 1;
    const int64_t owned = last_read >= first_read ? last_read - first_read + 1 : 0;
    tot->row0 = first_read - F / 4;
    tot->n_owned = owned;
    if (owned == 0) return;
    const int64_t row = last_read - F / 4;
    if (row >= P.qrows_cap) return;
    for (int ph = 1; ph <= 3; ph += 2) {
        const int64_t g = 4 * last_read + ph;
        if (g < F + n) continue;
        int64_t Fp = F + n;
        for (int p = rank + 1; p < nranks; ++p) {
            const int64_t np = all[p].n_lines;
            if (g < Fp + np) {
                const int64_t j = g - Fp;
                if (j < all[p].edge_n) {
                    if (ph == 1) { P.qrows[row].soff = all[p].edge_off[j]; P.qrows[row].rlen = all[p].edge_len[j]; }
                    else P.qrows[row].qoff = all[p].edge_off[j];
                }
                break;
            }
            Fp += np;
        }
    }
}

__global__ void __launch_bounds__(256) split_point_kernel(const uint8_t *file, int64_t n, int64_t from, int want_header,
                                                          long long *out) {
    __shared__ long long s_best;
    if (threadIdx.x == 0) s_best = LLONG_MAX;
    __syncthreads();
    if (from <= 0) {
        if (!want_header || (n > 0 && file[0] == '>')) { if (threadIdx.x == 0) *out = 0; return; }
        from = 1;
    }
    for (int64_t c0 = from - 1; c0 < n; c0 += 256 * 16) {
        const int64_t a = c0 + threadIdx.x * 16;
        long long mine = LLONG_MAX;
        for (int i = 0; i < 16; ++i) {
            const int64_t x = a + i;
            if (x < n && file[x] == '\n' && (!want_header || (x + 1 < n && file[x + 1] == '>'))) { mine = x + 1; break; }
        }
        if (mine != LLONG_MAX) atomicMin(&s_best, mine);
        __syncthreads();
        if (s_best != LLONG_MAX) break;
        __syncthreads();
    }
    if (threadIdx.x == 0) *out = s_best == LLONG_MAX ? n : s_best;
}

}

using namespace fxg;

static int64_t guess_rows(int mode, int64_t n) { return (mode == 0 ? n / 1024 : n / 200) + 4096; }

static int scan_params(fxg_ctx *ctx, const fxg_file *f, int mode, int64_t base_offset, int flags, bool reserve,
                       ScanParams *out, int64_t *tmp_slots) {
    const int64_t n = f->size;
    const int64_t nreg = (n + 1 + REGION - 1) / REGION;
    const int64_t nb = (nreg + PS_BLOCK - 1) / PS_BLOCK;
    const int64_t nreg_pad = nb * PS_BLOCK;
    const size_t off_bs = fxg_round_up((int64_t)nreg_pad * 8, 256);
    const size_t off_ex = off_bs + fxg_round_up(nb * (int64_t)sizeof(ulonglong2), 256);
    const size_t off_r2 = off_ex + fxg_round_up(nreg * (int64_t)sizeof(ulonglong2), 256);
    int rc;
    if (reserve) {
        if ((rc = ctx->counters.reserve(1024))) return rc;
        if ((rc = ctx->tile_desc.reserve(off_r2 + (mode == 0 ? (size_t)nreg * sizeof(uint4) : 0)))) return rc;
        if ((rc = ctx->seg.reserve((size_t)nreg * SEGCAP * sizeof(uint16_t)))) return rc;
        if (FXG_MARK_CUT && mode == 1 && (rc = ctx->cut.reserve((size_t)nreg * SEGCAP))) return rc;
        const int64_t want = guess_rows(mode, n);
        if (mode == 0) {
            if (ctx->row_tmp.cap < (size_t)(want + 2) * sizeof(FastaTmp) && (rc = ctx->row_tmp.reserve((size_t)(want + 2) * sizeof(FastaTmp)))) return rc;
            if (ctx->rows.cap < (size_t)(want + 1) * sizeof(fxg_fasta_row) && (rc = ctx->rows.reserve((size_t)(want + 1) * sizeof(fxg_fasta_row)))) return rc;
        } else if (ctx->rows.cap < (size_t)(want + 2) * sizeof(fxg_fastq_row)) {
            if ((rc = ctx->rows.reserve((size_t)(want + 2) * sizeof(fxg_fastq_row)))) return rc;
        }
    }
    ScanParams P;
    memset(&P, 0, sizeof(P));
    P.file = f->d; P.n = n; P.capacity = f->capacity & ~(int64_t)15; P.nreg = nreg;
    P.base_offset = base_offset; P.first_line = 0; P.flags = flags;
    P.rc = (uint2 *)ctx->tile_desc.ptr;
    P.bs = (ulonglong2 *)((uint8_t *)ctx->tile_desc.ptr + off_bs);
    P.ex = (ulonglong2 *)((uint8_t *)ctx->tile_desc.ptr + off_ex);
    P.rec2 = (uint4 *)((uint8_t *)ctx->tile_desc.ptr + off_r2);
    P.seg = (uint16_t *)ctx->seg.ptr;
    P.cut = (uint8_t *)ctx->cut.ptr;
    P.totals = (ScanTotals *)((uint8_t *)ctx->counters.ptr + 64);
    *tmp_slots = 0;
    if (mode == 0) {
        *tmp_slots = (int64_t)(ctx->row_tmp.cap / sizeof(FastaTmp));
        P.tmp = (FastaTmp *)ctx->row_tmp.ptr;
        P.tmp_cap = *tmp_slots - 1;
    } else {
        P.qrows = (fxg_fastq_row *)ctx->rows.ptr;
        P.qrows_cap = (int64_t)(ctx->rows.cap / sizeof(fxg_fastq_row));
    }
    *out = P;
    return FXG_OK;
}

static fxg_shard_info *own_info(fxg_ctx *ctx) { return (fxg_shard_info *)((uint8_t *)ctx->counters.ptr + 256); }

extern "C" int fxg_scan_begin(fxg_ctx *ctx, const fxg_file *f, int mode, int64_t base_offset, int flags,
                              fxg_shard_info *d_info_out) {
    FXG_CHECK_ARG(ctx && f && (mode == 0 || mode == 1), "null ctx/file or bad mode");
    FXG_LOCK(ctx);
    FXG_CUDA(cudaSetDevice(ctx->device));
    ctx->run.active = false;
    ScanParams P;
    int64_t tmp_slots;
    int rc = scan_params(ctx, f, mode, base_offset, flags, true, &P, &tmp_slots);
    if (rc) return rc;
    const int64_t n = f->size, nreg = P.nreg;
    const int64_t nb = (nreg + PS_BLOCK - 1) / PS_BLOCK, nreg_pad = nb * PS_BLOCK;
    FXG_CUDA(cudaMemsetAsync(ctx->counters.ptr, 0, 1024, ctx->stream));
    if (nreg_pad > nreg) FXG_CUDA(cudaMemsetAsync(P.rc + nreg, 0, (size_t)(nreg_pad - nreg) * 8, ctx->stream));
    const unsigned grid = (unsigned)((nreg + (int64_t)MARK_WARPS * FXG_MARK_RPW - 1) / ((int64_t)MARK_WARPS * FXG_MARK_RPW));
    {
        FxgProfScope prof(ctx, FXG_PROF_SCAN);
        if (mode == 0) mark_kernel<0, FXG_MARK_V_FASTA><<<grid, MARK_WARPS * 32, 0, ctx->stream>>>(P);
        else mark_kernel<1, FXG_MARK_V_FASTQ><<<grid, MARK_WARPS * 32, 0, ctx->stream>>>(P);
    }
    FXG_CUDA(cudaGetLastError());
    {
        FxgProfScope prof(ctx, FXG_PROF_PREFIX, 4);
        prefix_reduce_kernel<<<(unsigned)nb, PS_THREADS, 0, ctx->stream>>>(P.rc, P.bs);
        prefix_blocks_kernel<<<1, 1024, 0, ctx->stream>>>(P.bs, nb, P.file, n, mode, P.totals);
        prefix_expand_kernel<<<(unsigned)nb, PS_THREADS, 0, ctx->stream>>>(P.rc, P.bs, P.ex, nreg);
        edge_kernel<<<1, 32, 0, ctx->stream>>>(P, mode, own_info(ctx));
    }
    FXG_CUDA(cudaGetLastError());
    if (d_info_out)
        FXG_CUDA(cudaMemcpyAsync(d_info_out, own_info(ctx), sizeof(fxg_shard_info), cudaMemcpyDeviceToDevice, ctx->stream));
    ctx->run.active = true; ctx->run.mode = mode; ctx->run.flags = flags; ctx->run.file = f; ctx->run.base_offset = base_offset;
    return FXG_OK;
}

static int launch_phase_b(fxg_ctx *ctx, const ScanParams &P0, int mode, int64_t tmp_slots, const fxg_shard_info *d_all,
                          int nranks, int rank) {
    int rc0 = ctx->params.reserve(512);
    if (rc0) return rc0;
    if (!ctx->h_counters) FXG_CUDA(cudaHostAlloc(&ctx->h_counters, 8192, cudaHostAllocDefault));
    ScanParams P = P0;
    P.self = (const ScanParams *)ctx->params.ptr;
    static_assert(sizeof(ScanParams) <= 512, "ScanParams staging");
    memcpy((uint8_t *)ctx->h_counters + 4096, &P, sizeof(P));
    FXG_CUDA(cudaMemcpyAsync(ctx->params.ptr, (uint8_t *)ctx->h_counters + 4096, sizeof(P), cudaMemcpyHostToDevice, ctx->stream));
    const int64_t nreg = P.nreg;
    {
        FxgProfScope prof(ctx, FXG_PROF_LINES, 3);
        shard_prefix_kernel<<<1, 32, 0, ctx->stream>>>(d_all, nranks, rank, mode, P.totals);
        clear_kernel<<<ctx->sm_count * 4, 256, 0, ctx->stream>>>(P, mode, tmp_slots);
        if (mode == 0) {
            const unsigned lgrid = (unsigned)((nreg + MARK_WARPS * 32 - 1) / (MARK_WARPS * 32));
            fasta_lines_kernel<<<lgrid, MARK_WARPS * 32, 0, ctx->stream>>>(P);
        } else if (getenv("FXG_FASTQ_LINES_GENERIC")) {
            const unsigned lgrid = (unsigned)((nreg + MARK_WARPS * LG - 1) / (MARK_WARPS * LG));
            lines_kernel<1><<<lgrid, MARK_WARPS * 32, 0, ctx->stream>>>(P);
        } else {
            const unsigned lgrid = (unsigned)((nreg + MARK_WARPS * RG - 1) / (MARK_WARPS * RG));
            fastq_records_kernel<<<lgrid, MARK_WARPS * 32, 0, ctx->stream>>>(P);
        }
    }
    FXG_CUDA(cudaGetLastError());
    {
        FxgProfScope prof(ctx, FXG_PROF_FINALIZE);
        if (mode == 0)
            fasta_finalize_kernel<<<ctx->sm_count * 4, 256, 0, ctx->stream>>>(
                P.tmp, P.tmp_cap, (int64_t)(ctx->rows.cap / sizeof(fxg_fasta_row)), P.base_offset, P.totals,
                (fxg_fasta_row *)ctx->rows.ptr);
        else
            fastq_stitch_kernel<<<1, 32, 0, ctx->stream>>>(P, d_all, nranks, rank);
    }
    FXG_CUDA(cudaGetLastError());
    return FXG_OK;
}

extern "C" int fxg_scan_finish(fxg_ctx *ctx, const fxg_shard_info *d_all, int nranks, int rank, void **d_rows_out,
                               fxg_scan_stats *stats, fxg_shard_info *all_host) {
    FXG_CHECK_ARG(ctx && stats && nranks >= 1 && rank >= 0 && rank < nranks, "bad arguments");
    FXG_LOCK(ctx);
    FXG_CHECK_ARG(ctx->run.active, "fxg_scan_finish without fxg_scan_begin");
    FXG_CUDA(cudaSetDevice(ctx->device));
    ctx->run.active = false;
    const int mode = ctx->run.mode;
    const fxg_file *f = ctx->run.file;
    if (!d_all) { FXG_CHECK_ARG(nranks == 1, "d_all == NULL with more than one rank"); d_all = own_info(ctx); }
    memset(stats, 0, sizeof(*stats));
    if (d_rows_out) *d_rows_out = nullptr;
    if (!ctx->h_counters) FXG_CUDA(cudaHostAlloc(&ctx->h_counters, 8192, cudaHostAllocDefault));
    FXG_CHECK_ARG((size_t)nranks * sizeof(fxg_shard_info) + 256 <= 4096 || !all_host, "too many ranks for all_host");
    ScanTotals *ht = (ScanTotals *)ctx->h_counters;
    fxg_shard_info *hall = (fxg_shard_info *)((uint8_t *)ctx->h_counters + 256);
    for (int attempt = 0; attempt < 2; ++attempt) {
        ScanParams P;
        int64_t tmp_slots;
        int rc = scan_params(ctx, f, mode, ctx->run.base_offset, ctx->run.flags, false, &P, &tmp_slots);
        if (rc) return rc;
        if ((rc = launch_phase_b(ctx, P, mode, tmp_slots, d_all, nranks, rank))) return rc;
        FXG_CUDA(cudaMemcpyAsync(ht, P.totals, sizeof(ScanTotals), cudaMemcpyDeviceToHost, ctx->stream));
        if (all_host)
            FXG_CUDA(cudaMemcpyAsync(hall, d_all, (size_t)nranks * sizeof(fxg_shard_info), cudaMemcpyDeviceToHost, ctx->stream));
        FXG_CUDA(cudaStreamSynchronize(ctx->stream));
        bool fits;
        if (mode == 0) fits = ht->nrows + 2 <= tmp_slots && (size_t)(ht->nrows + 1) * sizeof(fxg_fasta_row) <= ctx->rows.cap;
        else fits = ht->nrows <= P.qrows_cap;
        if (fits) break;
        if (attempt == 1) { fxg_set_error("row buffers still too small after regrowing"); return FXG_ENOMEM; }
        if (mode == 0) {
            if ((rc = ctx->row_tmp.reserve((size_t)(ht->nrows + 2) * sizeof(FastaTmp)))) return rc;
            if ((rc = ctx->rows.reserve((size_t)(ht->nrows + 1) * sizeof(fxg_fasta_row)))) return rc;
        } else if ((rc = ctx->rows.reserve((size_t)(ht->nrows + 2) * sizeof(fxg_fastq_row)))) return rc;
    }
    stats->n_lines = (int64_t)ht->nl;
    stats->end_position = ht->n_eff;
    stats->total_len = (int64_t)ht->sum_len;
    if (mode == 0) {
        stats->n_rows = ht->nrows;
        stats->lead_llen = ht->lead_llen;
        if (ht->nrows > 0) { stats->lead_lines = ht->lead_lines; stats->lead_bytes = ht->lead_bytes; }
        else { stats->lead_lines = (int64_t)ht->nl; stats->lead_bytes = f->size; }
        if (d_rows_out) *d_rows_out = ctx->rows.ptr;
    } else {
        stats->n_rows = ht->n_owned;
        stats->lead_lines = ht->first_line;
        stats->reserved = ht->total_lines;
        if (d_rows_out) *d_rows_out = (fxg_fastq_row *)ctx->rows.ptr + ht->row0;
    }
    if (all_host) memcpy(all_host, hall, (size_t)nranks * sizeof(fxg_shard_info));
    return FXG_OK;
}

extern "C" int fxg_scan_sharded(fxg_ctx *ctx, fxg_comm *comm, const fxg_file *f, int mode, int64_t base_offset, int flags,
                                void **d_rows_out, fxg_scan_stats *stats, fxg_shard_info *all_host) {
    FXG_CHECK_ARG(ctx && f && stats, "null ctx/file/stats");
    FXG_LOCK(ctx);
    const int nranks = comm ? fxg_comm_nranks(comm) : 1, rank = comm ? fxg_comm_rank(comm) : 0;
    int rc = ctx->misc.reserve((size_t)nranks * sizeof(fxg_shard_info) + 256);
    if (rc) return rc;
    fxg_shard_info *d_all = (fxg_shard_info *)ctx->misc.ptr;
    if ((rc = fxg_scan_begin(ctx, f, mode, base_offset, flags, nullptr))) return rc;
    if ((rc = fxg_shard_exchange(ctx, comm, own_info(ctx), d_all, sizeof(fxg_shard_info)))) return rc;
    if ((rc = fxg_scan_finish(ctx, d_all, nranks, rank, d_rows_out, stats, all_host))) return rc;
    return comm ? fxg_comm_check(comm) : FXG_OK;
}

extern "C" int fxg_fasta_scan(fxg_ctx *ctx, const fxg_file *f, int64_t base_offset, int flags,
                              fxg_fasta_row **d_rows_out, fxg_scan_stats *stats) {
    FXG_CHECK_ARG(ctx && f && stats, "null ctx/file/stats");
    FXG_LOCK(ctx);
    int rc = fxg_scan_begin(ctx, f, 0, base_offset, flags, nullptr);
    if (rc) return rc;
    return fxg_scan_finish(ctx, nullptr, 1, 0, (void **)d_rows_out, stats, nullptr);
}

extern "C" int fxg_fastq_scan(fxg_ctx *ctx, const fxg_file *f, int64_t base_offset,
                              fxg_fastq_row **d_rows_out, fxg_scan_stats *stats) {
    FXG_CHECK_ARG(ctx && f && stats, "null ctx/file/stats");
    FXG_LOCK(ctx);
    int rc = fxg_scan_begin(ctx, f, 1, base_offset, 0, nullptr);
    if (rc) return rc;
    return fxg_scan_finish(ctx, nullptr, 1, 0, (void **)d_rows_out, stats, nullptr);
}

extern "C" int fxg_split_point_dev(fxg_ctx *ctx, const fxg_file *f, int64_t from, int want_header, int64_t *pos) {
    FXG_CHECK_ARG(ctx && f && pos && from >= 0, "bad arguments");
    FXG_LOCK(ctx);
    FXG_CUDA(cudaSetDevice(ctx->device));
    if (from >= f->size) { *pos = f->size; return FXG_OK; }
    int rc;
    if ((rc = ctx->counters.reserve(1024))) return rc;
    long long *d = (long long *)((uint8_t *)ctx->counters.ptr + 512);
    ctx->launches += 1;
    split_point_kernel<<<1, 256, 0, ctx->stream>>>(f->d, f->size, from, want_header, d);
    FXG_CUDA(cudaGetLastError());
    long long h = 0;
    FXG_CUDA(cudaMemcpyAsync(&h, d, 8, cudaMemcpyDeviceToHost, ctx->stream));
    FXG_CUDA(cudaStreamSynchronize(ctx->stream));
    *pos = (int64_t)h;
    return FXG_OK;
}
```

Before: 4552.

## Fuse FASTA prefix expansion and clearing into row kernel, compact line work per warp

Removes the per-region expand pass and separate clear kernel for FASTA by computing the exclusive line/header prefix inside the row kernel from per-span block sums. The span-level reduce kernel replaces the block-level one, and a single scan_edge kernel takes over the block prefix. The row kernel compacts line items into shared memory so all lanes process lines evenly. The tmp buffer is now zeroed by the finalize kernel for reuse instead of a clear kernel, and name search reads a wider window to avoid byte-by-byte fallback. This cuts launches and global traffic in exchange for more complex kernels and a persistent zeroed scratch invariant.

```diff
diff --git a/pyfastx_b200/csrc/fxg_api.cu b/pyfastx_b200/csrc/fxg_api.cu
--- a/pyfastx_b200/csrc/fxg_api.cu
+++ b/pyfastx_b200/csrc/fxg_api.cu
@@ -114,7 +114,7 @@
     for (int i = 0; i < FXG_PROF_SLOTS; ++i)
         for (int j = 0; j < 2; ++j) if (c->prof_ev[i][j]) cudaEventDestroy(c->prof_ev[i][j]);
     c->tile_desc.release(); c->seg.release(); c->cut.release(); c->row_tmp.release(); c->rows.release();
-    c->counters.release(); c->params.release(); c->plan.release(); c->misc.release(); c->stage_file.release();
+    c->counters.release(); c->params.release(); c->plan.release(); c->misc.release(); c->stage_file.release(); c->fasta_tmp.release();
     if (c->own_stream && c->stream) cudaStreamDestroy(c->stream);
     delete c;
 }
diff --git a/pyfastx_b200/csrc/fxg_common.cuh b/pyfastx_b200/csrc/fxg_common.cuh
--- a/pyfastx_b200/csrc/fxg_common.cuh
+++ b/pyfastx_b200/csrc/fxg_common.cuh
@@ -60,6 +60,7 @@
     void        *ring = nullptr;
     cudaEvent_t  ring_ev[32] = {};
     FxgScratch   tile_desc, seg, cut, row_tmp, rows, counters, params, plan, misc, stage_file;
+    FxgScratch   fasta_tmp;
     void        *h_counters = nullptr;
     void        *h_one = nullptr;
     void        *svc_req = nullptr, *svc_resp = nullptr;
diff --git a/pyfastx_b200/csrc/fxg_scan.cu b/pyfastx_b200/csrc/fxg_scan.cu
--- a/pyfastx_b200/csrc/fxg_scan.cu
+++ b/pyfastx_b200/csrc/fxg_scan.cu
@@ -12,6 +12,8 @@
 constexpr int SEGCAP   = 128;
 constexpr int MARK_WARPS = 8;
 constexpr int PS_THREADS = 256, PS_PER_THREAD = 16, PS_BLOCK = PS_THREADS * PS_PER_THREAD;
+constexpr int SPAN = MARK_WARPS * 32;
+static_assert(PS_BLOCK % SPAN == 0 && SPAN == 16 * PS_PER_THREAD, "a span is one half-warp of the reduce kernel");
 constexpr int64_t NOPOS = INT64_MIN / 4;
 constexpr uint32_t E_POS = 0x07ffu, E_CR = 1u << 14, E_HDR = 1u << 15;
 
@@ -355,8 +357,8 @@
 }
 
 __global__ void __launch_bounds__(PS_THREADS) prefix_reduce_kernel(const uint2 *rc, ulonglong2 *bs) {
-    __shared__ uint32_t sm[16];
-    const uint4 *p = reinterpret_cast<const uint4 *>(rc + (size_t)blockIdx.x * PS_BLOCK + (size_t)threadIdx.x * PS_PER_THREAD);
+    const size_t t = (size_t)blockIdx.x * PS_THREADS + threadIdx.x;
+    const uint4 *p = reinterpret_cast<const uint4 *>(rc + t * PS_PER_THREAD);
     uint32_t a = 0, b = 0;
 #pragma unroll
     for (int i = 0; i < PS_PER_THREAD / 2; ++i) {
@@ -364,55 +366,16 @@
         a += (q.x & 0xffffu) + (q.z & 0xffffu);
         b += (q.x >> 16) + (q.z >> 16);
     }
-    a = __reduce_add_sync(0xffffffffu, a);
-    b = __reduce_add_sync(0xffffffffu, b);
-    const int lane = threadIdx.x & 31, warp = threadIdx.x >> 5;
-    if (lane == 0) { sm[warp] = a; sm[8 + warp] = b; }
-    __syncthreads();
-    if (threadIdx.x == 0) {
-        uint64_t ta = 0, tb = 0;
-        for (int w = 0; w < PS_THREADS / 32; ++w) { ta += sm[w]; tb += sm[8 + w]; }
-        bs[blockIdx.x] = make_ulonglong2(ta, tb);
-    }
-}
-
-__global__ void __launch_bounds__(1024) prefix_blocks_kernel(ulonglong2 *bs, int64_t nb, const uint8_t *file, int64_t n,
-                                                             int mode, ScanTotals *tot) {
-    __shared__ uint64_t s_a[32], s_b[32];
-    __shared__ uint64_t s_ca, s_cb;
-    const int lane = threadIdx.x & 31, warp = threadIdx.x >> 5;
-    if (threadIdx.x == 0) { s_ca = 0; s_cb = (mode == 0 && n > 0 && file[0] == '>') ? 1u : 0u; }
-    __syncthreads();
-    for (int64_t b0 = 0; b0 < nb; b0 += 1024) {
-        const int64_t i = b0 + threadIdx.x;
-        const ulonglong2 v = i < nb ? bs[i] : make_ulonglong2(0, 0);
-        uint64_t a = v.x, b = v.y;
-#pragma unroll
-        for (int d = 1; d < 32; d <<= 1) {
-            const uint64_t oa = (uint64_t)shfl_up_i64((int64_t)a, d), ob = (uint64_t)shfl_up_i64((int64_t)b, d);
-            if (lane >= d) { a += oa; b += ob; }
-        }
-        if (lane == 31) { s_a[warp] = a; s_b[warp] = b; }
-        __syncthreads();
-        uint64_t wa = 0, wb = 0;
-        for (int w = 0; w < warp; ++w) { wa += s_a[w]; wb += s_b[w]; }
-        const uint64_t ca = s_ca, cb = s_cb;
-        if (i < nb) bs[i] = make_ulonglong2(ca + wa + a - v.x, cb + wb + b - v.y);
-        __syncthreads();
-        if (threadIdx.x == 1023) { s_ca = ca + wa + a; s_cb = cb + wb + b; }
-        __syncthreads();
-    }
-    if (threadIdx.x == 0) {
-        const bool virt = n > 0 && file[n - 1] != '\n';
-        tot->nl = s_ca; tot->hdr = s_cb; tot->n_eff = n + (virt ? 1 : 0);
-    }
+#pragma unroll
+    for (int d = 8; d > 0; d >>= 1) { a += __shfl_xor_sync(0xffffffffu, a, d); b += __shfl_xor_sync(0xffffffffu, b, d); }
+    if ((threadIdx.x & 15) == 0) bs[t / 16] = make_ulonglong2(a, b);
 }
 
 __global__ void __launch_bounds__(PS_THREADS) prefix_expand_kernel(const uint2 *rc, const ulonglong2 *bs, ulonglong2 *ex,
                                                                  int64_t nreg) {
-    __shared__ uint32_t s_a[PS_THREADS / 32], s_b[PS_THREADS / 32];
-    const int lane = threadIdx.x & 31, warp = threadIdx.x >> 5;
-    const size_t r0 = (size_t)blockIdx.x * PS_BLOCK + (size_t)threadIdx.x * PS_PER_THREAD;
+    const int sub = threadIdx.x & 15;
+    const size_t t = (size_t)blockIdx.x * PS_THREADS + threadIdx.x;
+    const size_t r0 = t * PS_PER_THREAD;
     const uint4 *p = reinterpret_cast<const uint4 *>(rc + r0);
     uint32_t c[PS_PER_THREAD];
     uint32_t a = 0, b = 0;
@@ -425,16 +388,12 @@
     }
     uint32_t ia = a, ib = b;
 #pragma unroll
-    for (int d = 1; d < 32; d <<= 1) {
-        const uint32_t oa = __shfl_up_sync(0xffffffffu, ia, d), ob = __shfl_up_sync(0xffffffffu, ib, d);
-        if (lane >= d) { ia += oa; ib += ob; }
-    }
-    if (lane == 31) { s_a[warp] = ia; s_b[warp] = ib; }
-    __syncthreads();
-    uint32_t wa = 0, wb = 0;
-    for (int w = 0; w < warp; ++w) { wa += s_a[w]; wb += s_b[w]; }
-    const ulonglong2 bb = bs[blockIdx.x];
-    uint64_t ea = bb.x + wa + ia - a, eb = bb.y + wb + ib - b;
+    for (int d = 1; d < 16; d <<= 1) {
+        const uint32_t oa = __shfl_up_sync(0xffffffffu, ia, d, 16), ob = __shfl_up_sync(0xffffffffu, ib, d, 16);
+        if (sub >= d) { ia += oa; ib += ob; }
+    }
+    const ulonglong2 bb = bs[t / 16];
+    uint64_t ea = bb.x + ia - a, eb = bb.y + ib - b;
 #pragma unroll
     for (int i = 0; i < PS_PER_THREAD; ++i) {
         if ((int64_t)(r0 + i) < nreg) ex[r0 + i] = make_ulonglong2(ea, eb);
@@ -494,9 +453,10 @@
             int64_t nlen = dlen;
             if (!(P.flags & FXG_SCAN_FULL_NAME)) {
                 nlen = 0;
-                if (s + 1 + dlen + 20 <= P.capacity) {
+                if (s + 1 + (L - 2) + 20 <= P.capacity) {
                     int which;
-                    nlen = find_first_of2(file + s + 1, dlen, 0x20202020u, 0x09090909u, &which);
+                    nlen = find_first_of2(file + s + 1, L - 2, 0x20202020u, 0x09090909u, &which);
+                    if (nlen > dlen) nlen = dlen;
                 } else {
                     while (nlen < dlen) {
                         const uint8_t ch = file[s + 1 + nlen];
@@ -684,13 +644,13 @@
 }
 
 template <int MODE>
-__device__ __noinline__ unsigned long long full_region(const ScanParams *Pg, int64_t first_line, int64_t r) {
+__device__ __noinline__ unsigned long long full_region(const ScanParams *Pg, int64_t first_line, int64_t r, ulonglong2 X) {
     const ScanParams &P = *Pg;
     unsigned long long my_size = 0;
     const int lane = threadIdx.x & 31;
     const int nl = (int)(P.rc[r].x & 0xffffu);
     if (nl == 0) return 0;
-    const ulonglong2 X = P.ex[r];
+    if (MODE == 1) X = P.ex[r];
     Prev2 cy = carry_walk<MODE>(Pg, r);
     if (MODE != 0) cy.h1 = cy.h0 = 0;
     if (nl <= SEGCAP) region_batches<MODE>(P, first_line, r, nl, cy, X, P.seg[r * SEGCAP + lane], P.seg[r * SEGCAP + 32 + lane], my_size);
@@ -802,7 +762,7 @@
     const uint32_t densem = __ballot_sync(0xffffffffu, nll > (uint32_t)SEGCAP);
     if (densem & (((1u << RG) - 1u) << 1)) {
         for (int i = 0; i < RG; ++i)
-            if (r0 + i < P.nreg) my_size += full_region<1>(P.self, first_line, r0 + i);
+            if (r0 + i < P.nreg) my_size += full_region<1>(P.self, first_line, r0 + i, make_ulonglong2(0, 0));
     } else {
         const uint64_t ex0 = (uint64_t)shfl_i64((int64_t)exl, 1);
         uint16_t *flat = s_flat[warp];
@@ -942,23 +902,39 @@
     if (lane == 0 && my_size) atomicAdd((unsigned long long *)&P.totals->sum_len, my_size);
 }
 
-__global__ void __launch_bounds__(MARK_WARPS * 32) fasta_lines_kernel(const ScanParams P) {
-    const int lane = threadIdx.x & 31;
-    const int64_t R0 = ((int64_t)blockIdx.x * MARK_WARPS + (threadIdx.x >> 5)) * 32;
-    if (R0 >= P.nreg) return;
+__global__ void __launch_bounds__(SPAN) fasta_rows_kernel(const ScanParams P) {
+    __shared__ uint32_t s_a[MARK_WARPS], s_b[MARK_WARPS];
+    __shared__ uint16_t s_item[MARK_WARPS][32 * 32];
+    const int lane = threadIdx.x & 31, warp = threadIdx.x >> 5;
+    const int64_t R0 = (int64_t)blockIdx.x * SPAN + warp * 32;
     const int64_t r = R0 + lane;
     const bool inb = r < P.nreg;
-    unsigned long long dummy = 0;
-    uint2 me = make_uint2(0u, 0u), pv = make_uint2(0u, 0u);
+    if (blockIdx.x == 0 && threadIdx.x == 0) {
+        P.totals->nrows = (int64_t)P.totals->hdr;
+        P.totals->sum_len = 0;
+    }
+    const uint2 me = P.rc[r];
+    const ulonglong2 sb = P.bs[blockIdx.x];
+    uint2 pv = make_uint2(0u, 0u);
     uint4 q = make_uint4(0u, 0u, 0u, 0u);
-    ulonglong2 X = make_ulonglong2(0, 0);
     if (inb) {
-        me = P.rc[r];
         if (r >= 1) pv = P.rc[r - 1];
         q = P.rec2[r];
-        X = P.ex[r];
-    }
-    const uint32_t nl = me.x & 0xffffu, pnl = pv.x & 0xffffu;
+    }
+    const uint32_t nl = me.x & 0xffffu, hc = me.x >> 16, pnl = pv.x & 0xffffu;
+    uint32_t ia = nl, ib = hc;
+#pragma unroll
+    for (int d = 1; d < 32; d <<= 1) {
+        const uint32_t oa = __shfl_up_sync(0xffffffffu, ia, d), ob = __shfl_up_sync(0xffffffffu, ib, d);
+        if (lane >= d) { ia += oa; ib += ob; }
+    }
+    if (lane == 31) { s_a[warp] = ia; s_b[warp] = ib; }
+    __syncthreads();
+    if (R0 >= P.nreg) return;
+    for (int w = 0; w < warp; ++w) { ia += s_a[w]; ib += s_b[w]; }
+    const ulonglong2 X = make_ulonglong2(sb.x + ia - nl, sb.y + ib - hc);
+
+    unsigned long long dummy = 0;
     const bool full = nl != 0 && (nl > 32u || r == 0 || pnl < 2u || pnl > (uint32_t)SEGCAP || q.y == 0xffffffffu);
     uint32_t mask = 0;
     const uint32_t c1 = pv.y & 0xffffu, c0 = pv.y >> 16, f0 = q.x & 0xffffu, f1 = q.x >> 16;
@@ -971,111 +947,188 @@
         mask = (q.y & ~3u) | (i0 ? 1u : 0u) | (i1 ? 2u : 0u);
         if (nl < 32u) mask &= (1u << nl) - 1u;
     }
-    const int64_t base = r * REGION;
-    const uint16_t *sg = P.seg + r * SEGCAP;
-    while (mask) {
-        const int k = __ffs(mask) - 1;
-        mask &= mask - 1;
+    uint32_t incl = (uint32_t)__popc(mask);
+#pragma unroll
+    for (int d = 1; d < 32; d <<= 1) {
+        const uint32_t o = __shfl_up_sync(0xffffffffu, incl, d);
+        if (lane >= d) incl += o;
+    }
+    const uint32_t total = __shfl_sync(0xffffffffu, incl, 31);
+    uint16_t *items = s_item[warp];
+    for (uint32_t o = incl - (uint32_t)__popc(mask), m = mask; m; m &= m - 1) items[o++] = (uint16_t)((lane << 5) | (__ffs(m) - 1));
+    __syncwarp();
+    for (uint32_t t0 = 0; t0 < total; t0 += 32) {
+        const uint32_t t = t0 + (uint32_t)lane;
+        const uint32_t it = t < total ? (uint32_t)items[t] : 0u;
+        const int src = (int)(it >> 5), k = (int)(it & 31u);
+        const uint32_t sx = __shfl_sync(0xffffffffu, q.x, src), sz = __shfl_sync(0xffffffffu, q.z, src);
+        const uint32_t sy = __shfl_sync(0xffffffffu, pv.y, src);
+        const int64_t xx = shfl_i64((int64_t)X.x, src), xy = shfl_i64((int64_t)X.y, src);
+        if (t >= total) continue;
+        const uint32_t g1 = sy & 0xffffu, g0 = sy >> 16, h0 = sx & 0xffffu, h1 = sx >> 16;
+        const int64_t base = (R0 + src) * REGION;
+        const uint16_t *sg = P.seg + (R0 + src) * SEGCAP;
         uint32_t e, m1, m2;
         int64_t b1 = base, b2 = base;
         if (k >= 2) { e = sg[k]; m1 = sg[k - 1]; m2 = sg[k - 2]; }
-        else if (k == 1) { e = f1; m1 = f0; m2 = c1; b2 = base - REGION; }
-        else { e = f0; m1 = c1; m2 = c0; b1 = b2 = base - REGION; }
+        else if (k == 1) { e = h1; m1 = h0; m2 = g1; b2 = base - REGION; }
+        else { e = h0; m1 = g1; m2 = g0; b1 = b2 = base - REGION; }
         do_line<0>(P, 0, base + (e & E_POS), b1 + (m1 & E_POS), b2 + (m2 & E_POS), (m1 & E_HDR) != 0, (m2 & E_HDR) != 0,
-                   (int64_t)X.y + __popc(q.z & ((1u << k) - 1u)), (int64_t)X.x + k, false, dummy);
+                   xy + __popc(sz & ((1u << k) - 1u)), xx + k, false, dummy);
     }
     uint32_t fm = __ballot_sync(0xffffffffu, full);
     while (fm) {
         const int f = __ffs(fm) - 1;
         fm &= fm - 1;
-        full_region<0>(P.self, 0, R0 + f);
-    }
-}
-
-
-__global__ void __launch_bounds__(256) fasta_finalize_kernel(const FastaTmp *tmp, int64_t tmp_cap, int64_t rows_cap,
+        const ulonglong2 Xf = make_ulonglong2((uint64_t)shfl_i64((int64_t)X.x, f), (uint64_t)shfl_i64((int64_t)X.y, f));
+        full_region<0>(P.self, 0, R0 + f, Xf);
+    }
+}
+
+
+__global__ void __launch_bounds__(256) fasta_finalize_kernel(FastaTmp *tmp, int64_t tmp_cap, int64_t rows_cap,
                                                              int64_t base_offset, ScanTotals *tot, fxg_fasta_row *rows) {
-    int64_t nrows = (int64_t)tot->hdr;
-    if (nrows > rows_cap || nrows + 1 > tmp_cap) nrows = 0;
+    const int64_t hdr = (int64_t)tot->hdr;
+    const int64_t nslots = hdr + 1 < tmp_cap ? hdr + 1 : tmp_cap;
+    const bool fits = hdr <= rows_cap && hdr + 1 <= tmp_cap;
     unsigned long long slen_acc = 0;
     const int64_t stride = (int64_t)gridDim.x * blockDim.x;
-    for (int64_t r = (int64_t)blockIdx.x * blockDim.x + threadIdx.x; r < nrows; r += stride) {
-        const FastaTmp t = tmp[r + 1];
-        int64_t next_h, next_line;
-        if (r + 1 < nrows) {
-            const FastaTmp nx = tmp[r + 2];
-            next_h = nx.boff - (1 + nx.dlen + (int64_t)nx.elen);
-            next_line = nx.lineidx;
-        } else {
-            next_h = base_offset + tot->n_eff;
-            next_line = (int64_t)tot->nl;
-        }
-        const int64_t blen = next_h - t.boff;
-        const int64_t nlines = next_line - t.lineidx - 1;
-        const int64_t slen = blen - nlines * (int64_t)t.elen;
-        int norm;
-        if (t.D == 0) norm = 1;
-        else if (t.D == 1) norm = ((int64_t)t.evmax == t.lineidx + nlines) ? 1 : 0;
-        else if (t.D == 2) norm = ((t.evmax - (~t.evminc) == 1) && t.S == 0) ? 1 : 0;
-        else norm = 0;
-        fxg_fasta_row o;
-        o.boff = t.boff; o.blen = blen; o.slen = slen; o.llen = t.llen;
-        o.dlen = t.dlen; o.nlen = t.nlen; o.elen = (uint8_t)t.elen; o.norm = (uint8_t)norm;
-        for (int i = 0; i < 6; ++i) o.pad[i] = 0;
-        o.pad[0] = (t.D == 0 || (t.D == 1 && (int64_t)t.evmax == t.lineidx + nlines && (int64_t)t.S < 0)) ? 1 : 0;
-        rows[r] = o;
-        slen_acc += (unsigned long long)slen;
+    for (int64_t sl = (int64_t)blockIdx.x * blockDim.x + threadIdx.x; sl < nslots; sl += stride) {
+        const FastaTmp t = tmp[sl];
+        if (sl == 0) {
+            tot->lead_llen = t.llen;
+            if (fits && hdr > 0) {
+                const FastaTmp *f = &tmp[1];
+                tot->lead_lines = f->lineidx;
+                tot->lead_bytes = f->boff - base_offset - (1 + f->dlen + (int64_t)f->elen);
+            }
+        } else if (fits) {
+            const int64_t r = sl - 1;
+            int64_t next_h, next_line;
+            if (sl < hdr) {
+                const FastaTmp *nx = &tmp[sl + 1];
+                next_h = nx->boff - (1 + nx->dlen + (int64_t)nx->elen);
+                next_line = nx->lineidx;
+            } else {
+                next_h = base_offset + tot->n_eff;
+                next_line = (int64_t)tot->nl;
+            }
+            const int64_t blen = next_h - t.boff;
+            const int64_t nlines = next_line - t.lineidx - 1;
+            const int64_t slen = blen - nlines * (int64_t)t.elen;
+            int norm;
+            if (t.D == 0) norm = 1;
+            else if (t.D == 1) norm = ((int64_t)t.evmax == t.lineidx + nlines) ? 1 : 0;
+            else if (t.D == 2) norm = ((t.evmax - (~t.evminc) == 1) && t.S == 0) ? 1 : 0;
+            else norm = 0;
+            fxg_fasta_row o;
+            o.boff = t.boff; o.blen = blen; o.slen = slen; o.llen = t.llen;
+            o.dlen = t.dlen; o.nlen = t.nlen; o.elen = (uint8_t)t.elen; o.norm = (uint8_t)norm;
+            for (int i = 0; i < 6; ++i) o.pad[i] = 0;
+            o.pad[0] = (t.D == 0 || (t.D == 1 && (int64_t)t.evmax == t.lineidx + nlines && (int64_t)t.S < 0)) ? 1 : 0;
+            rows[r] = o;
+            slen_acc += (unsigned long long)slen;
+        }
+        FastaTmp *z = &tmp[sl];
+        z->llen = 0; z->S = 0; z->evmax = 0; z->evminc = 0; z->D = 0;
     }
 #pragma unroll
     for (int d = 16; d > 0; d >>= 1) slen_acc += (unsigned long long)shfl_down_i64((int64_t)slen_acc, d);
     if ((threadIdx.x & 31) == 0 && slen_acc) atomicAdd((unsigned long long *)&tot->sum_len, slen_acc);
-    if (blockIdx.x == 0 && threadIdx.x == 0) {
-        const FastaTmp l = tmp[0];
-        tot->lead_llen = l.llen;
-        if (nrows > 0) {
-            const FastaTmp f = tmp[1];
-            tot->lead_lines = f.lineidx;
-            tot->lead_bytes = f.boff - base_offset - (1 + f.dlen + (int64_t)f.elen);
-        }
-    }
-}
-
-__global__ void __launch_bounds__(32) edge_kernel(const ScanParams P, int mode, fxg_shard_info *info) {
-    const int lane = threadIdx.x;
+}
+
+__global__ void __launch_bounds__(1024) scan_edge_kernel(const ScanParams P, int64_t nspan, int mode, fxg_shard_info *info) {
+    __shared__ uint64_t s_a[32], s_b[32], s_nl, s_hdr;
+    const int lane = threadIdx.x & 31, warp = threadIdx.x >> 5;
+    ulonglong2 *bs = P.bs;
+    constexpr int SB = 8;
+    const int64_t per = (nspan + 31) / 32;
+    const int64_t i0 = min(nspan, (int64_t)warp * per), i1 = min(nspan, i0 + per);
+    auto load_steps = [&](int64_t i, ulonglong2 (&v)[SB]) {
+#pragma unroll
+        for (int j = 0; j < SB; ++j) {
+            const int64_t k = i + 32 * j + lane;
+            v[j] = k < i1 ? bs[k] : make_ulonglong2(0, 0);
+        }
+    };
+    uint64_t a = 0, b = 0;
+    for (int64_t i = i0; i < i1; i += 32 * SB) {
+        ulonglong2 v[SB];
+        load_steps(i, v);
+#pragma unroll
+        for (int j = 0; j < SB; ++j) { a += v[j].x; b += v[j].y; }
+    }
+
     int found = 0;
-    int64_t pos[3] = {0, 0, 0};
-    for (int64_t r0 = 0; r0 < P.nreg && found < 3; r0 += 32) {
-        const int64_t r = r0 + lane;
-        const uint32_t c = r < P.nreg ? (P.rc[r].x & 0xffffu) : 0u;
-        uint32_t nz = __ballot_sync(0xffffffffu, c != 0);
-        while (nz && found < 3) {
-            const int fl = __ffs(nz) - 1;
-            nz &= nz - 1;
-            const int64_t q = r0 + fl;
-            const int cq = (int)__shfl_sync(0xffffffffu, c, fl);
-            if (cq <= SEGCAP) {
-                for (int i = 0; i < cq && found < 3; ++i) pos[found++] = q * REGION + (int64_t)(P.seg[q * SEGCAP + i] & E_POS);
-            } else {
-                for (int64_t x = q * REGION; x < q * REGION + REGION && found < 3; ++x)
-                    if (nl_at(P, x)) pos[found++] = x;
-            }
-        }
-    }
-    if (lane == 0) {
-        const ScanTotals t = *P.totals;
+    int64_t pos0 = 0, pos1 = 0, pos2 = 0;
+    auto push = [&](int64_t x) { if (found == 0) pos0 = x; else if (found == 1) pos1 = x; else pos2 = x; ++found; };
+    if (warp == 0) {
+        for (int64_t r0 = 0; r0 < P.nreg && found < 3; r0 += 32) {
+            const int64_t r = r0 + lane;
+            const uint32_t c = r < P.nreg ? (P.rc[r].x & 0xffffu) : 0u;
+            uint32_t nz = __ballot_sync(0xffffffffu, c != 0);
+            while (nz && found < 3) {
+                const int fl = __ffs(nz) - 1;
+                nz &= nz - 1;
+                const int64_t q = r0 + fl;
+                const int cq = (int)__shfl_sync(0xffffffffu, c, fl);
+                if (cq <= SEGCAP) {
+                    for (int i = 0; i < cq && found < 3; ++i) push(q * REGION + (int64_t)(P.seg[q * SEGCAP + i] & E_POS));
+                } else {
+                    for (int64_t x = q * REGION; x < q * REGION + REGION && found < 3; ++x)
+                        if (nl_at(P, x)) push(x);
+                }
+            }
+        }
+    }
+
+#pragma unroll
+    for (int d = 16; d > 0; d >>= 1) {
+        a += (uint64_t)shfl_down_i64((int64_t)a, d);
+        b += (uint64_t)shfl_down_i64((int64_t)b, d);
+    }
+    if (lane == 0) { s_a[warp] = a; s_b[warp] = b; }
+    __syncthreads();
+    const int64_t n = P.n;
+    uint64_t ca = 0, cb = (mode == 0 && n > 0 && P.file[0] == '>') ? 1u : 0u;
+    for (int w = 0; w < warp; ++w) { ca += s_a[w]; cb += s_b[w]; }
+    for (int64_t i = i0; i < i1; i += 32 * SB) {
+        ulonglong2 v[SB];
+        load_steps(i, v);
+#pragma unroll
+        for (int j = 0; j < SB; ++j) {
+            uint64_t xa = v[j].x, xb = v[j].y;
+#pragma unroll
+            for (int d = 1; d < 32; d <<= 1) {
+                const uint64_t oa = (uint64_t)shfl_up_i64((int64_t)xa, d), ob = (uint64_t)shfl_up_i64((int64_t)xb, d);
+                if (lane >= d) { xa += oa; xb += ob; }
+            }
+            const int64_t k = i + 32 * j + lane;
+            if (k < i1) bs[k] = make_ulonglong2(ca + xa - v[j].x, cb + xb - v[j].y);
+            ca += (uint64_t)shfl_i64((int64_t)xa, 31); cb += (uint64_t)shfl_i64((int64_t)xb, 31);
+        }
+    }
+    if (threadIdx.x == 1023) {
+        ScanTotals *tot = P.totals;
+        tot->nl = ca; tot->hdr = cb;
+        tot->n_eff = n + ((n > 0 && P.file[n - 1] != '\n') ? 1 : 0);
+        s_nl = ca; s_hdr = cb;
+    }
+    __syncthreads();
+    if (threadIdx.x == 0) {
         fxg_shard_info o;
-        o.n_rows = mode == 0 ? (int64_t)t.hdr : 0;
-        o.n_lines = (int64_t)t.nl;
-        o.bytes = P.n;
+        o.n_rows = mode == 0 ? (int64_t)s_hdr : 0;
+        o.n_lines = (int64_t)s_nl;
+        o.bytes = n;
         o.base_offset = P.base_offset;
-        o.end_position = t.n_eff;
+        o.end_position = n + ((n > 0 && P.file[n - 1] != '\n') ? 1 : 0);
         o.edge_n = found;
         int64_t start = 0;
         for (int j = 0; j < 3; ++j) {
             o.edge_off[j] = 0; o.edge_len[j] = 0;
             if (j < found) {
-                const int64_t p = pos[j];
-                const bool cr = p > start && p - 1 < P.n && P.file[p - 1] == '\r';
+                const int64_t p = j == 0 ? pos0 : (j == 1 ? pos1 : pos2);
+                const bool cr = p > start && p - 1 < n && P.file[p - 1] == '\r';
                 o.edge_off[j] = P.base_offset + start;
                 o.edge_len[j] = p - start - (cr ? 1 : 0);
                 start = p + 1;
@@ -1086,7 +1139,7 @@
     }
 }
 
-__global__ void shard_prefix_kernel(const fxg_shard_info *all, int nranks, int rank, int mode, ScanTotals *tot) {
+__global__ void shard_prefix_kernel(const fxg_shard_info *all, int nranks, int rank, ScanTotals *tot) {
     if (threadIdx.x != 0 || blockIdx.x != 0) return;
     int64_t F = 0, T = 0;
     for (int p = 0; p < nranks; ++p) {
@@ -1094,24 +1147,17 @@
         if (p < rank) F += nlp;
         T += nlp;
     }
-    if (mode == 0) F = 0;
     tot->first_line = F;
     tot->total_lines = T;
     const int64_t nl = (int64_t)tot->nl;
-    tot->nrows = mode == 0 ? (int64_t)tot->hdr : (F + nl + 3) / 4 - F / 4;
+    tot->nrows = (F + nl + 3) / 4 - F / 4;
     tot->sum_len = 0;
 }
 
-__global__ void __launch_bounds__(256) clear_kernel(const ScanParams P, int mode, int64_t tmp_slots) {
+__global__ void __launch_bounds__(32) clear_kernel(const ScanParams P) {
     const int64_t nrows = P.totals->nrows;
-    const int64_t stride = (int64_t)gridDim.x * blockDim.x;
-    const int64_t t0 = (int64_t)blockIdx.x * blockDim.x + threadIdx.x;
-    if (mode == 0) {
-        int64_t slots = nrows + 2;
-        if (slots > tmp_slots) slots = tmp_slots;
-        uint4 *p = reinterpret_cast<uint4 *>(P.tmp);
-        for (int64_t i = t0; i < slots * 4; i += stride) p[i] = make_uint4(0u, 0u, 0u, 0u);
-    } else if (t0 < 4) {
+    const int t0 = threadIdx.x;
+    if (t0 < 4) {
         const int64_t row = t0 < 2 ? 0 : nrows - 1;
         if (row >= 0 && row < P.qrows_cap) reinterpret_cast<uint4 *>(P.qrows + row)[t0 & 1] = make_uint4(0u, 0u, 0u, 0u);
     }
@@ -1179,6 +1225,15 @@
 
 static int64_t guess_rows(int mode, int64_t n) { return (mode == 0 ? n / 1024 : n / 200) + 4096; }
 
+static int reserve_fasta_tmp(fxg_ctx *ctx, int64_t slots) {
+    const size_t bytes = (size_t)slots * sizeof(FastaTmp);
+    if (bytes <= ctx->fasta_tmp.cap) return FXG_OK;
+    int rc = ctx->fasta_tmp.reserve(bytes);
+    if (rc) return rc;
+    FXG_CUDA(cudaMemsetAsync(ctx->fasta_tmp.ptr, 0, ctx->fasta_tmp.cap, ctx->stream));
+    return FXG_OK;
+}
+
 static int scan_params(fxg_ctx *ctx, const fxg_file *f, int mode, int64_t base_offset, int flags, bool reserve,
                        ScanParams *out, int64_t *tmp_slots) {
     const int64_t n = f->size;
@@ -1186,8 +1241,8 @@
     const int64_t nb = (nreg + PS_BLOCK - 1) / PS_BLOCK;
     const int64_t nreg_pad = nb * PS_BLOCK;
     const size_t off_bs = fxg_round_up((int64_t)nreg_pad * 8, 256);
-    const size_t off_ex = off_bs + fxg_round_up(nb * (int64_t)sizeof(ulonglong2), 256);
-    const size_t off_r2 = off_ex + fxg_round_up(nreg * (int64_t)sizeof(ulonglong2), 256);
+    const size_t off_ex = off_bs + fxg_round_up(nreg_pad / SPAN * (int64_t)sizeof(ulonglong2), 256);
+    const size_t off_r2 = off_ex + (mode == 1 ? fxg_round_up(nreg * (int64_t)sizeof(ulonglong2), 256) : 0);
     int rc;
     if (reserve) {
         if ((rc = ctx->counters.reserve(1024))) return rc;
@@ -1196,7 +1251,7 @@
         if (FXG_MARK_CUT && mode == 1 && (rc = ctx->cut.reserve((size_t)nreg * SEGCAP))) return rc;
         const int64_t want = guess_rows(mode, n);
         if (mode == 0) {
-            if (ctx->row_tmp.cap < (size_t)(want + 2) * sizeof(FastaTmp) && (rc = ctx->row_tmp.reserve((size_t)(want + 2) * sizeof(FastaTmp)))) return rc;
+            if ((rc = reserve_fasta_tmp(ctx, want + 2))) return rc;
             if (ctx->rows.cap < (size_t)(want + 1) * sizeof(fxg_fasta_row) && (rc = ctx->rows.reserve((size_t)(want + 1) * sizeof(fxg_fasta_row)))) return rc;
         } else if (ctx->rows.cap < (size_t)(want + 2) * sizeof(fxg_fastq_row)) {
             if ((rc = ctx->rows.reserve((size_t)(want + 2) * sizeof(fxg_fastq_row)))) return rc;
@@ -1208,15 +1263,15 @@
     P.base_offset = base_offset; P.first_line = 0; P.flags = flags;
     P.rc = (uint2 *)ctx->tile_desc.ptr;
     P.bs = (ulonglong2 *)((uint8_t *)ctx->tile_desc.ptr + off_bs);
-    P.ex = (ulonglong2 *)((uint8_t *)ctx->tile_desc.ptr + off_ex);
-    P.rec2 = (uint4 *)((uint8_t *)ctx->tile_desc.ptr + off_r2);
+    P.ex = mode == 1 ? (ulonglong2 *)((uint8_t *)ctx->tile_desc.ptr + off_ex) : nullptr;
+    P.rec2 = mode == 0 ? (uint4 *)((uint8_t *)ctx->tile_desc.ptr + off_r2) : nullptr;
     P.seg = (uint16_t *)ctx->seg.ptr;
     P.cut = (uint8_t *)ctx->cut.ptr;
     P.totals = (ScanTotals *)((uint8_t *)ctx->counters.ptr + 64);
     *tmp_slots = 0;
     if (mode == 0) {
-        *tmp_slots = (int64_t)(ctx->row_tmp.cap / sizeof(FastaTmp));
-        P.tmp = (FastaTmp *)ctx->row_tmp.ptr;
+        *tmp_slots = (int64_t)(ctx->fasta_tmp.cap / sizeof(FastaTmp));
+        P.tmp = (FastaTmp *)ctx->fasta_tmp.ptr;
         P.tmp_cap = *tmp_slots - 1;
     } else {
         P.qrows = (fxg_fastq_row *)ctx->rows.ptr;
@@ -1238,7 +1293,7 @@
     int64_t tmp_slots;
     int rc = scan_params(ctx, f, mode, base_offset, flags, true, &P, &tmp_slots);
     if (rc) return rc;
-    const int64_t n = f->size, nreg = P.nreg;
+    const int64_t nreg = P.nreg;
     const int64_t nb = (nreg + PS_BLOCK - 1) / PS_BLOCK, nreg_pad = nb * PS_BLOCK;
     FXG_CUDA(cudaMemsetAsync(ctx->counters.ptr, 0, 1024, ctx->stream));
     if (nreg_pad > nreg) FXG_CUDA(cudaMemsetAsync(P.rc + nreg, 0, (size_t)(nreg_pad - nreg) * 8, ctx->stream));
@@ -1250,11 +1305,10 @@
     }
     FXG_CUDA(cudaGetLastError());
     {
-        FxgProfScope prof(ctx, FXG_PROF_PREFIX, 4);
+        FxgProfScope prof(ctx, FXG_PROF_PREFIX, mode == 0 ? 2 : 3);
         prefix_reduce_kernel<<<(unsigned)nb, PS_THREADS, 0, ctx->stream>>>(P.rc, P.bs);
-        prefix_blocks_kernel<<<1, 1024, 0, ctx->stream>>>(P.bs, nb, P.file, n, mode, P.totals);
-        prefix_expand_kernel<<<(unsigned)nb, PS_THREADS, 0, ctx->stream>>>(P.rc, P.bs, P.ex, nreg);
-        edge_kernel<<<1, 32, 0, ctx->stream>>>(P, mode, own_info(ctx));
+        scan_edge_kernel<<<1, 1024, 0, ctx->stream>>>(P, nreg_pad / SPAN, mode, own_info(ctx));
+        if (mode == 1) prefix_expand_kernel<<<(unsigned)nb, PS_THREADS, 0, ctx->stream>>>(P.rc, P.bs, P.ex, nreg);
     }
     FXG_CUDA(cudaGetLastError());
     if (d_info_out)
@@ -1263,7 +1317,7 @@
     return FXG_OK;
 }
 
-static int launch_phase_b(fxg_ctx *ctx, const ScanParams &P0, int mode, int64_t tmp_slots, const fxg_shard_info *d_all,
+static int launch_phase_b(fxg_ctx *ctx, const ScanParams &P0, int mode, const fxg_shard_info *d_all,
                           int nranks, int rank) {
     int rc0 = ctx->params.reserve(512);
     if (rc0) return rc0;
@@ -1275,18 +1329,19 @@
     FXG_CUDA(cudaMemcpyAsync(ctx->params.ptr, (uint8_t *)ctx->h_counters + 4096, sizeof(P), cudaMemcpyHostToDevice, ctx->stream));
     const int64_t nreg = P.nreg;
     {
-        FxgProfScope prof(ctx, FXG_PROF_LINES, 3);
-        shard_prefix_kernel<<<1, 32, 0, ctx->stream>>>(d_all, nranks, rank, mode, P.totals);
-        clear_kernel<<<ctx->sm_count * 4, 256, 0, ctx->stream>>>(P, mode, tmp_slots);
+        FxgProfScope prof(ctx, FXG_PROF_LINES, mode == 0 ? 1 : 3);
         if (mode == 0) {
-            const unsigned lgrid = (unsigned)((nreg + MARK_WARPS * 32 - 1) / (MARK_WARPS * 32));
-            fasta_lines_kernel<<<lgrid, MARK_WARPS * 32, 0, ctx->stream>>>(P);
-        } else if (getenv("FXG_FASTQ_LINES_GENERIC")) {
-            const unsigned lgrid = (unsigned)((nreg + MARK_WARPS * LG - 1) / (MARK_WARPS * LG));
-            lines_kernel<1><<<lgrid, MARK_WARPS * 32, 0, ctx->stream>>>(P);
+            fasta_rows_kernel<<<(unsigned)((nreg + SPAN - 1) / SPAN), SPAN, 0, ctx->stream>>>(P);
         } else {
-            const unsigned lgrid = (unsigned)((nreg + MARK_WARPS * RG - 1) / (MARK_WARPS * RG));
-            fastq_records_kernel<<<lgrid, MARK_WARPS * 32, 0, ctx->stream>>>(P);
+            shard_prefix_kernel<<<1, 32, 0, ctx->stream>>>(d_all, nranks, rank, P.totals);
+            clear_kernel<<<1, 32, 0, ctx->stream>>>(P);
+            if (getenv("FXG_FASTQ_LINES_GENERIC")) {
+                const unsigned lgrid = (unsigned)((nreg + MARK_WARPS * LG - 1) / (MARK_WARPS * LG));
+                lines_kernel<1><<<lgrid, MARK_WARPS * 32, 0, ctx->stream>>>(P);
+            } else {
+                const unsigned lgrid = (unsigned)((nreg + MARK_WARPS * RG - 1) / (MARK_WARPS * RG));
+                fastq_records_kernel<<<lgrid, MARK_WARPS * 32, 0, ctx->stream>>>(P);
+            }
         }
     }
     FXG_CUDA(cudaGetLastError());
@@ -1324,7 +1379,7 @@
         int64_t tmp_slots;
         int rc = scan_params(ctx, f, mode, ctx->run.base_offset, ctx->run.flags, false, &P, &tmp_slots);
         if (rc) return rc;
-        if ((rc = launch_phase_b(ctx, P, mode, tmp_slots, d_all, nranks, rank))) return rc;
+        if ((rc = launch_phase_b(ctx, P, mode, d_all, nranks, rank))) return rc;
         FXG_CUDA(cudaMemcpyAsync(ht, P.totals, sizeof(ScanTotals), cudaMemcpyDeviceToHost, ctx->stream));
         if (all_host)
             FXG_CUDA(cudaMemcpyAsync(hall, d_all, (size_t)nranks * sizeof(fxg_shard_info), cudaMemcpyDeviceToHost, ctx->stream));
@@ -1335,7 +1390,7 @@
         if (fits) break;
         if (attempt == 1) { fxg_set_error("row buffers still too small after regrowing"); return FXG_ENOMEM; }
         if (mode == 0) {
-            if ((rc = ctx->row_tmp.reserve((size_t)(ht->nrows + 2) * sizeof(FastaTmp)))) return rc;
+            if ((rc = reserve_fasta_tmp(ctx, ht->nrows + 2))) return rc;
             if ((rc = ctx->rows.reserve((size_t)(ht->nrows + 1) * sizeof(fxg_fasta_row)))) return rc;
         } else if ((rc = ctx->rows.reserve((size_t)(ht->nrows + 2) * sizeof(fxg_fastq_row)))) return rc;
     }
```

New measurement: 4638, median of 6. 1.9% higher.
